# ErlerPhilipp/points2surf

Hardware: NVIDIA B200
Metric: SDF queries/sec at grid_res=256 (higher is better)
Workload: dtype f16 operands / f32 accumulate (tcgen05); hi/lo split f16 (fp32-level) for FC tails and guard-band recompute

## Files before the change

points2surf_b200/csrc/net_tc.cu:

```cuda
#include "model.cuh"
#include "tc_ptx.cuh"

#ifndef P2S_TC_BOUNDED_WAIT
#define P2S_TC_BOUNDED_WAIT 1
#endif

namespace p2s {

using namespace ptx;

namespace {

constexpr int kTile = 128;
constexpr int kThreads = 576;
constexpr uint32_t kAct2Bytes = 32768;
constexpr uint32_t kSmallBytes = 192 * 4 + 320 * 4 + 168;
template <bool PRECISE>
struct Cfg {
    static constexpr int kChunks = PRECISE ? 1 : 4;
    static constexpr int kSplit = 8 / kChunks;
    static constexpr uint32_t kChunkBytes = PRECISE ? 65536u : 32768u;
    static constexpr uint32_t kW3Bytes = kChunks * kChunkBytes;
    static constexpr uint32_t kMidBytes = (8192u + 8192u + 16384u) * (PRECISE ? 2u : 1u);
    static constexpr uint32_t kOffMid = kW3Bytes;
    static constexpr uint32_t kOffAct2 = kOffMid + kMidBytes;
    static constexpr uint32_t kOffSmall = kOffAct2 + 2 * kAct2Bytes;
    static constexpr uint32_t kSmemBytes = kOffSmall + kSmallBytes;
    static constexpr uint32_t kACols = PRECISE ? 64u : 32u;
    static constexpr uint32_t kPerqBytes = PRECISE ? 16384u : 8192u;
    static constexpr uint32_t kMidScale = PRECISE ? 2u : 1u;
};
static_assert(Cfg<false>::kSmemBytes <= 232448 && Cfg<true>::kSmemBytes <= 232448, "shared memory budget");
constexpr uint32_t kColD3 = 0;
constexpr uint32_t kColDmid = 256;
constexpr uint32_t kColDmidB = 448;
constexpr uint32_t kColA = 384;

struct Seg {
    const float* ptr;
    int n;
    int tiles;
    int center;
};

struct PassParams {
    Seg seg[2];
    const float* query;
    const float* R;
    int tiles_per_query;
    int B;
    const float* W0;
    const float* b0;
    int num_mid;
    int mid_N[3];
    const uint8_t* mid_img[3];
    const float* mid_bias[3];
    int perq_layer;
    const uint8_t* perq_img;
    const uint8_t* w3_img;
    float* out;
    long long* wstats;
};

struct Bars {
    uint64_t w_full, wq_full, perq_done;
    uint64_t dmid_free[2];
    uint64_t a_ready[2], a_free[2], dmid_ready[2];
    uint64_t act2_full[2], act2_empty[2], d3_full[2], d3_empty[2];
    uint32_t tmem_base;
};
static_assert(sizeof(Bars) <= 168, "barrier block");

__device__ __forceinline__ void wait_bar(uint64_t* bar, uint32_t parity, long long* acc = nullptr) {
#if P2S_TC_BOUNDED_WAIT
    long long t0 = clock64();
    while (!mbar_try_wait(bar, parity)) {
        if (clock64() - t0 > 2000000000LL) {
            printf("p2s: mbarrier timeout block %d thread %d bar %p parity %u\n", blockIdx.x, threadIdx.x, (void*)bar, parity);
            __trap();
        }
    }
    if (acc) *acc += clock64() - t0;
#else
    mbar_wait(bar, parity);
#endif
}
enum { WS_ACT2_FULL = 0, WS_D3_EMPTY, WS_DMID_FREE, WS_DMID_READY, WS_ACT2_EMPTY, WS_A_FREE, WS_D3_FULL, WS_TOTAL, WS_SLOTS };
__device__ __forceinline__ void ws_flush(long long* g, int role, const long long* ws, long long t_begin) {
    if (!g || (threadIdx.x & 31) != 0) return;
    for (int i = 0; i < WS_TOTAL; ++i) if (ws[i]) atomicAdd((unsigned long long*)&g[role * WS_SLOTS + i], (unsigned long long)ws[i]);
    atomicAdd((unsigned long long*)&g[role * WS_SLOTS + WS_TOTAL], (unsigned long long)(clock64() - t_begin));
}

__device__ __forceinline__ uint32_t pack_relu(float a, float b) {
    uint32_t r;
    asm("cvt.rn.relu.satfinite.f16x2.f32 %0, %1, %2;" : "=r"(r) : "f"(b), "f"(a));
    return r;
}
__device__ __forceinline__ void pack_relu_split(float a, float b, uint32_t& hi, uint32_t& lo) {
    hi = pack_relu(a, b);
    const float2 hf = __half22float2(*reinterpret_cast<const __half2*>(&hi));
    lo = pack_half2(fmaxf(a, 0.f) - hf.x, fmaxf(b, 0.f) - hf.y);
}

template <bool PRECISE, bool STATS = false>
__global__ void __launch_bounds__(kThreads, 1) pointnet_pass_kernel(const PassParams p) {
    using C = Cfg<PRECISE>;
    constexpr uint32_t kOffMid = C::kOffMid, kOffAct2 = C::kOffAct2, kOffSmall = C::kOffSmall, kOffW3 = 0;
    extern __shared__ __align__(1024) uint8_t smem[];
    float* s_wq = reinterpret_cast<float*>(smem + kOffSmall);
    float* s_bias = s_wq + 192;
    Bars* bars = reinterpret_cast<Bars*>(s_bias + 320);
    const int tid = threadIdx.x, warp = tid >> 5, lane = tid & 31;
    const int part = blockIdx.x % C::kSplit;
    const int stream = blockIdx.x / C::kSplit, nstreams = gridDim.x / C::kSplit;
    const int nq = (p.B > stream) ? (p.B - stream + nstreams - 1) / nstreams : 0;
    const int tpq = p.tiles_per_query;
    const int ntiles = nq * tpq;

    if (tid == 0) {
        mbar_init(&bars->w_full, 1);
        mbar_init(&bars->wq_full, 1);
        mbar_init(&bars->perq_done, 1);
        mbar_init(&bars->dmid_free[0], 128);
        mbar_init(&bars->dmid_free[1], 128);
        for (int i = 0; i < 2; ++i) {
            mbar_init(&bars->a_ready[i], 128);
            mbar_init(&bars->a_free[i], 128);
            mbar_init(&bars->dmid_ready[i], 1);
            mbar_init(&bars->act2_full[i], 128);
            mbar_init(&bars->act2_empty[i], 1);
            mbar_init(&bars->d3_full[i], 1);
            mbar_init(&bars->d3_empty[i], 128);
        }
        fence_mbar_init();
    }
    if (warp == 8) { tmem_alloc(&bars->tmem_base, 512); tmem_relinquish(); }
    {
        int off = 0;
        for (int l = 0; l < p.num_mid; ++l) {
            for (int i = tid; i < p.mid_N[l]; i += kThreads) s_bias[off + i] = p.mid_bias[l][i];
            off += p.mid_N[l];
        }
        for (int i = tid; i < 64; i += kThreads) s_bias[256 + i] = p.b0[i];
    }
    tc_fence_before();
    __syncthreads();
    tc_fence_after();
    const uint32_t tmem = bars->tmem_base;
    long long ws[WS_TOTAL] = {0, 0, 0, 0, 0, 0, 0};
    long long* const wsp = STATS ? ws : nullptr;
    const long long t_begin = STATS ? clock64() : 0;

    if (warp == 8) {
        if (ntiles > 0) {
            if (lane == 0) {
                uint32_t bytes = C::kW3Bytes;
                for (int l = 0; l < p.num_mid; ++l) if (l != p.perq_layer) bytes += (uint32_t)p.mid_N[l] * 128u * C::kMidScale;
                mbar_arrive_expect_tx(&bars->w_full, bytes);
                for (uint32_t o = 0; o < C::kW3Bytes; o += 32768u)
                    bulk_g2s(smem + kOffW3 + o, p.w3_img + (size_t)part * C::kW3Bytes + o, 32768, &bars->w_full);
                uint32_t o = 0;
                for (int l = 0; l < p.num_mid; ++l) {
                    const uint32_t lb = (uint32_t)p.mid_N[l] * 128u * C::kMidScale;
                    if (l != p.perq_layer) bulk_g2s(smem + kOffMid + o, p.mid_img[l], lb, &bars->w_full);
                    else {
                        mbar_arrive_expect_tx(&bars->wq_full, C::kPerqBytes);
                        bulk_g2s(smem + kOffMid + o, p.perq_img + (size_t)stream * C::kPerqBytes, C::kPerqBytes, &bars->wq_full);
                    }
                    o += lb;
                }
            }
            __syncwarp();
            wait_bar(&bars->w_full, 0);
            const uint32_t idesc_l3 = make_idesc_f16(128, 128);
            const uint64_t dsc_w3 = make_smem_desc(smem_u32(smem + kOffW3), 128, 2048);
            const uint64_t dsc_act2 = make_smem_desc(smem_u32(smem + kOffAct2), 128, 2048);
            for (int it = 0; it < ntiles; ++it) {
                const uint32_t buf = PRECISE ? 0u : ((uint32_t)it & 1), buse = PRECISE ? (uint32_t)it : ((uint32_t)it >> 1);
                wait_bar(&bars->act2_full[buf], buse & 1, wsp ? wsp + WS_ACT2_FULL : nullptr);
                const uint64_t db = dsc_act2 + (uint64_t)(buf * (kAct2Bytes >> 4));
#pragma unroll
                for (int c = 0; c < C::kChunks; ++c) {
                    const uint32_t g = (uint32_t)(it * C::kChunks + c);
                    const uint32_t stage = g & 1, use = g >> 1;
                    wait_bar(&bars->d3_empty[stage], (use & 1) ^ 1, wsp ? wsp + WS_D3_EMPTY : nullptr);
                    tc_fence_after();
                    if (elect_one()) {
                        const uint64_t da = dsc_w3 + (uint64_t)((uint32_t)c * (C::kChunkBytes >> 4));
                        const uint32_t d = tmem + kColD3 + stage * 128u;
                        if (PRECISE) {
                            const uint64_t da_lo = da + (uint64_t)(32768u >> 4), db_lo = db + (uint64_t)(32768u >> 4);
#pragma unroll
                            for (int ks = 0; ks < 8; ++ks) {
                                mma_ss(d, da_lo + (uint64_t)(ks * 16), db + (uint64_t)(ks * 16), idesc_l3, ks > 0);
                                mma_ss(d, da + (uint64_t)(ks * 16), db_lo + (uint64_t)(ks * 16), idesc_l3, 1);
                                mma_ss(d, da + (uint64_t)(ks * 16), db + (uint64_t)(ks * 16), idesc_l3, 1);
                            }
                        } else {
#pragma unroll
                            for (int ks = 0; ks < 8; ++ks)
                                mma_ss(d, da + (uint64_t)(ks * 16), db + (uint64_t)(ks * 16), idesc_l3, ks > 0);
                        }
                        mma_commit(&bars->d3_full[stage]);
                        if (c == C::kChunks - 1) mma_commit(&bars->act2_empty[buf]);
                    }
                    __syncwarp();
                }
            }
        }
    } else if (warp == 13) {
        if (ntiles > 0) {
            uint32_t mid_off[3] = {0, 0, 0};
            {
                uint32_t o = 0;
                for (int l = 0; l < p.num_mid; ++l) { mid_off[l] = o; o += (uint32_t)p.mid_N[l] * 128u * C::kMidScale; }
            }
            const bool perq = p.perq_layer >= 0;
            wait_bar(&bars->w_full, 0);
            if (perq) wait_bar(&bars->wq_full, 0);
            const uint64_t dsc_mid0 = make_smem_desc(smem_u32(smem + kOffMid) + mid_off[0], 128, 1024);
            const uint64_t dsc_mid1 = make_smem_desc(smem_u32(smem + kOffMid) + mid_off[1], 128, 1024);
            const uint64_t dsc_mid2 = make_smem_desc(smem_u32(smem + kOffMid) + mid_off[2], 128, 1024);
            const uint32_t idesc_mid0 = make_idesc_f16(128, (uint32_t)p.mid_N[0]);
            const uint32_t idesc_mid1 = make_idesc_f16(128, (uint32_t)(p.num_mid > 1 ? p.mid_N[1] : 64));
            const uint32_t idesc_mid2 = make_idesc_f16(128, (uint32_t)(p.num_mid > 2 ? p.mid_N[2] : 64));
            int it_mid0 = 0, it_mid1 = 1, l_mid0 = 0, l_mid1 = 0;
            uint32_t rnd0 = 0, rnd1 = 0;
            uint32_t g_mid = 0;
            uint32_t g_buf0 = 0, g_buf1 = 0;
            int loaded_q = 0, perq_count = 0;
            bool pq_loading = false;
            while (it_mid0 < ntiles || it_mid1 < ntiles) {
                if (perq) {
                    if (!pq_loading && perq_count == tpq && loaded_q + 1 < nq && mbar_test_wait_warp(&bars->perq_done, (uint32_t)loaded_q & 1)) {
                        if (elect_one()) {
                            mbar_arrive_expect_tx(&bars->wq_full, C::kPerqBytes);
                            bulk_g2s(smem + kOffMid + mid_off[p.perq_layer],
                                     p.perq_img + ((size_t)stream + (size_t)(loaded_q + 1) * nstreams) * C::kPerqBytes, C::kPerqBytes, &bars->wq_full);
                        }
                        __syncwarp();
                        pq_loading = true;
                    }
                    if (pq_loading && mbar_test_wait_warp(&bars->wq_full, (uint32_t)(loaded_q + 1) & 1)) {
                        ++loaded_q; perq_count = 0; pq_loading = false;
                    }
                }
                auto try_mid = [&](const int c, int& it_m, int& l_m, uint32_t& rn) {
                    if (it_m >= ntiles) return;
                    const int l = l_m;
                    if (l == p.perq_layer && it_m / tpq != loaded_q) return;
                    if (!mbar_test_wait_warp(&bars->a_ready[c], rn & 1)) return;
                    const bool small = !PRECISE && (p.mid_N[l] == 64);
                    uint32_t& g_buf = small ? g_buf1 : g_buf0;
                    if (g_buf > 0) wait_bar(&bars->dmid_free[small ? 1 : 0], (g_buf - 1) & 1, wsp ? wsp + WS_DMID_FREE : nullptr);
                    tc_fence_after();
                    const uint32_t idesc = l == 0 ? idesc_mid0 : (l == 1 ? idesc_mid1 : idesc_mid2);
                    const uint64_t dsc = l == 0 ? dsc_mid0 : (l == 1 ? dsc_mid1 : dsc_mid2);
                    const uint32_t a_t = tmem + kColA + (uint32_t)c * C::kACols;
                    const uint32_t d_t = tmem + (small ? kColDmidB : kColDmid);
                    const bool pq_last = (l == p.perq_layer) && (perq_count + 1 == tpq);
                    if (elect_one()) {
                        if (PRECISE) {
                            const uint64_t dsc_lo = dsc + (uint64_t)(((uint32_t)p.mid_N[l] * 128u) >> 4);
#pragma unroll
                            for (int ks = 0; ks < 4; ++ks) {
                                mma_ts(d_t, a_t + 32 + ks * 8, dsc + (uint64_t)(ks * 16), idesc, ks > 0);
                                mma_ts(d_t, a_t + ks * 8, dsc_lo + (uint64_t)(ks * 16), idesc, 1);
                                mma_ts(d_t, a_t + ks * 8, dsc + (uint64_t)(ks * 16), idesc, 1);
                            }
                        } else {
#pragma unroll
                            for (int ks = 0; ks < 4; ++ks)
                                mma_ts(d_t, a_t + ks * 8, dsc + (uint64_t)(ks * 16), idesc, ks > 0);
                        }
                        mma_commit(&bars->dmid_ready[c]);
                        if (pq_last) mma_commit(&bars->perq_done);
                    }
                    __syncwarp();
                    ++g_mid; ++g_buf; ++rn;
                    if (l == p.perq_layer) ++perq_count;
                    if (++l_m == p.num_mid) { l_m = 0; it_m += 2; }
                };
                if (g_mid & 1) { try_mid(1, it_mid1, l_mid1, rnd1); try_mid(0, it_mid0, l_mid0, rnd0); }
                else { try_mid(0, it_mid0, l_mid0, rnd0); try_mid(1, it_mid1, l_mid1, rnd1); }
            }
        }
    } else if (warp < 4 || (warp >= 9 && warp < 13)) {
        const int c = (warp < 4) ? 0 : 1;
        const int grp = warp & 3;
        const int pt = grp * 32 + lane;
        const uint32_t lane_base = (uint32_t)(grp * 32) << 16;
        const uint32_t a_col = tmem + lane_base + kColA + (uint32_t)c * C::kACols;
        uint32_t round = 0;
        for (int it = c; it < ntiles; it += 2) {
            const uint32_t ab = PRECISE ? 0u : (uint32_t)c;
            const uint32_t au = PRECISE ? (uint32_t)it : ((uint32_t)it >> 1);
            int boff = 0;
            for (int l = 0; l < p.num_mid; ++l, ++round) {
                wait_bar(&bars->dmid_ready[c], round & 1, wsp ? wsp + WS_DMID_READY : nullptr);
                tc_fence_after();
                const int N = p.mid_N[l];
                const bool last = (l == p.num_mid - 1);
                if (last) {
                    tc_fence_before();
                    mbar_arrive(&bars->a_free[c]);
                }
                const bool small = !PRECISE && (N == 64);
                const uint32_t dcol = small ? kColDmidB : kColDmid;
                for (int n0 = 0; n0 < N; n0 += 32) {
                    uint32_t r[32];
                    tmem_ld_x32(tmem + lane_base + dcol + n0, r);
                    tmem_ld_wait();
                    if (n0 + 32 >= N) {
                        tc_fence_before();
                        mbar_arrive(&bars->dmid_free[small ? 1 : 0]);
                    }
                    uint32_t v[16], vl[16];
#pragma unroll
                    for (int j4 = 0; j4 < 8; ++j4) {
                        const float4 bb = *reinterpret_cast<const float4*>(s_bias + boff + n0 + 4 * j4);
                        const float2 s01 = fadd2(make_float2(__uint_as_float(r[4 * j4]), __uint_as_float(r[4 * j4 + 1])), make_float2(bb.x, bb.y));
                        const float2 s23 = fadd2(make_float2(__uint_as_float(r[4 * j4 + 2]), __uint_as_float(r[4 * j4 + 3])), make_float2(bb.z, bb.w));
                        if (PRECISE) {
                            pack_relu_split(s01.x, s01.y, v[2 * j4], vl[2 * j4]);
                            pack_relu_split(s23.x, s23.y, v[2 * j4 + 1], vl[2 * j4 + 1]);
                        } else {
                            v[2 * j4] = pack_relu(s01.x, s01.y);
                            v[2 * j4 + 1] = pack_relu(s23.x, s23.y);
                        }
                    }
                    if (!last) {
                        uint32_t w[8];
#pragma unroll
                        for (int h = 0; h < 2; ++h) {
#pragma unroll
                            for (int j = 0; j < 8; ++j) w[j] = v[h * 8 + j];
                            tmem_st_x8(a_col + (uint32_t)(n0 / 2 + h * 8), w);
                            if (PRECISE) {
#pragma unroll
                                for (int j = 0; j < 8; ++j) w[j] = vl[h * 8 + j];
                                tmem_st_x8(a_col + 32u + (uint32_t)(n0 / 2 + h * 8), w);
                            }
                        }
                    } else {
                        uint8_t* dst = smem + kOffAct2 + ab * kAct2Bytes + (uint32_t)(pt >> 3) * 2048u + (uint32_t)(pt & 7) * 16u;
#pragma unroll
                        for (int j = 0; j < 4; ++j) {
                            *reinterpret_cast<uint4*>(dst + (uint32_t)(n0 / 8 + j) * 128u) = make_uint4(v[4 * j], v[4 * j + 1], v[4 * j + 2], v[4 * j + 3]);
                            if (PRECISE)
                                *reinterpret_cast<uint4*>(dst + kAct2Bytes + (uint32_t)(n0 / 8 + j) * 128u) = make_uint4(vl[4 * j], vl[4 * j + 1], vl[4 * j + 2], vl[4 * j + 3]);
                        }
                    }
                }
                if (!last) {
                    tmem_st_wait();
                    if (l == p.num_mid - 2) wait_bar(&bars->act2_empty[ab], (au & 1) ^ 1, wsp ? wsp + WS_ACT2_EMPTY : nullptr);
                    tc_fence_before();
                    mbar_arrive(&bars->a_ready[c]);
                } else {
                    fence_proxy_async_smem();
                    tc_fence_before();
                    mbar_arrive(&bars->act2_full[ab]);
                }
                boff += N;
            }
        }
    } else if (warp >= 14) {
        const int grp = warp & 3;
        const int pt = grp * 32 + lane;
        const int ct = tid - 14 * 32;
        const uint32_t lane_base = (uint32_t)(grp * 32) << 16;
        float* wq = s_wq;
        const float* s_b0 = s_bias + 256;
        int cur_q = -1;
        auto fetch = [&](int it2, float& x, float& y, float& z, float& cx, float& cy, float& cz) {
            const int qi2 = it2 / tpq, tq2 = it2 - qi2 * tpq;
            const size_t q2 = (size_t)stream + (size_t)qi2 * nstreams;
            const int sgi = tq2 < p.seg[0].tiles ? 0 : 1;
            const Seg& sg = p.seg[sgi];
            int local = (tq2 - (sgi ? p.seg[0].tiles : 0)) * kTile + pt;
            if (local >= sg.n) local = 0;
            const float* src = sg.ptr + (q2 * sg.n + local) * 3;
            x = src[0]; y = src[1]; z = src[2];
            cx = cy = cz = 0.f;
            if (sg.center) { cx = p.query[q2 * 3 + 0]; cy = p.query[q2 * 3 + 1]; cz = p.query[q2 * 3 + 2]; }
        };
        float x = 0.f, y = 0.f, z = 0.f, pcx = 0.f, pcy = 0.f, pcz = 0.f;
        if (ntiles > 0) fetch(0, x, y, z, pcx, pcy, pcz);
        for (int it = 0; it < ntiles; ++it) {
            const int c = it & 1;
            const int qi = it / tpq;
            if (qi != cur_q) {
                const size_t q = (size_t)stream + (size_t)qi * nstreams;
                asm volatile("bar.sync 3, 128;" ::: "memory");
                if (ct < 64) {
                    float w0 = p.W0[ct * 3 + 0], w1 = p.W0[ct * 3 + 1], w2 = p.W0[ct * 3 + 2];
                    float r[9] = {1.f, 0.f, 0.f, 0.f, 1.f, 0.f, 0.f, 0.f, 1.f};
                    if (p.R) {
#pragma unroll
                        for (int i = 0; i < 9; ++i) r[i] = p.R[q * 9 + i];
                    }
                    wq[0 * 64 + ct] = w0 * r[0] + w1 * r[3] + w2 * r[6];
                    wq[1 * 64 + ct] = w0 * r[1] + w1 * r[4] + w2 * r[7];
                    wq[2 * 64 + ct] = w0 * r[2] + w1 * r[5] + w2 * r[8];
                }
                asm volatile("bar.sync 3, 128;" ::: "memory");
                cur_q = qi;
            }
            x -= pcx; y -= pcy; z -= pcz;
            uint32_t v[32], vl[PRECISE ? 32 : 1];
#pragma unroll
            for (int j4 = 0; j4 < 16; ++j4) {
                const float4 wx = *reinterpret_cast<const float4*>(wq + 0 * 64 + 4 * j4);
                const float4 wy = *reinterpret_cast<const float4*>(wq + 1 * 64 + 4 * j4);
                const float4 wz = *reinterpret_cast<const float4*>(wq + 2 * 64 + 4 * j4);
                const float4 bb = *reinterpret_cast<const float4*>(s_b0 + 4 * j4);
                const float2 xx = make_float2(x, x), yy = make_float2(y, y), zz = make_float2(z, z);
                const float2 h01 = ffma2(make_float2(wx.x, wx.y), xx, ffma2(make_float2(wy.x, wy.y), yy, ffma2(make_float2(wz.x, wz.y), zz, make_float2(bb.x, bb.y))));
                const float2 h23 = ffma2(make_float2(wx.z, wx.w), xx, ffma2(make_float2(wy.z, wy.w), yy, ffma2(make_float2(wz.z, wz.w), zz, make_float2(bb.z, bb.w))));
                if (PRECISE) {
                    pack_relu_split(h01.x, h01.y, v[2 * j4], vl[2 * j4]);
                    pack_relu_split(h23.x, h23.y, v[2 * j4 + 1], vl[2 * j4 + 1]);
                } else {
                    v[2 * j4] = pack_relu(h01.x, h01.y);
                    v[2 * j4 + 1] = pack_relu(h23.x, h23.y);
                }
            }
            if (it + 1 < ntiles) fetch(it + 1, x, y, z, pcx, pcy, pcz);
            wait_bar(&bars->a_free[c], (((uint32_t)it >> 1) & 1) ^ 1, wsp ? wsp + WS_A_FREE : nullptr);
            tc_fence_after();
            tmem_st_x32(tmem + lane_base + kColA + (uint32_t)c * C::kACols, v);
            if (PRECISE) {
                uint32_t (&vl32)[32] = reinterpret_cast<uint32_t (&)[32]>(vl);
                tmem_st_x32(tmem + lane_base + kColA + (uint32_t)c * C::kACols + 32u, vl32);
            }
            tmem_st_wait();
            if (p.num_mid == 1) wait_bar(&bars->act2_empty[PRECISE ? 0 : c], ((PRECISE ? (uint32_t)it : ((uint32_t)it >> 1)) & 1) ^ 1, wsp ? wsp + WS_ACT2_EMPTY : nullptr);
            tc_fence_before();
            mbar_arrive(&bars->a_ready[c]);
        }
    } else {
        const int ew = warp - 4;
        const uint32_t lane_base = (uint32_t)(ew * 32) << 16;
        const int ch_lane = ew * 32 + lane;
        int it = 0;
        for (int qi = 0; qi < nq; ++qi) {
            const int q = stream + qi * nstreams;
            float acc[C::kChunks];
#pragma unroll
            for (int c = 0; c < C::kChunks; ++c) acc[c] = -INFINITY;
            for (int tq = 0; tq < tpq; ++tq, ++it) {
#pragma unroll
                for (int c = 0; c < C::kChunks; ++c) {
                    const uint32_t g = (uint32_t)(it * C::kChunks + c);
                    const uint32_t stage = g & 1, use = g >> 1;
                    wait_bar(&bars->d3_full[stage], use & 1, wsp ? wsp + WS_D3_FULL : nullptr);
                    tc_fence_after();
                    const uint32_t d = tmem + lane_base + kColD3 + stage * 128u;
                    float m = acc[c];
#pragma unroll
                    for (int n0 = 0; n0 < 128; n0 += 64) {
                        uint32_t r0[32], r1[32];
                        tmem_ld_x32(d + n0, r0);
                        tmem_ld_x32(d + n0 + 32, r1);
                        tmem_ld_wait();
                        if (n0 == 64) {
                            tc_fence_before();
                            mbar_arrive(&bars->d3_empty[stage]);
                        }
#pragma unroll
                        for (int j = 0; j < 32; j += 2) m = fmax3(m, __uint_as_float(r0[j]), __uint_as_float(r0[j + 1]));
#pragma unroll
                        for (int j = 0; j < 32; j += 2) m = fmax3(m, __uint_as_float(r1[j]), __uint_as_float(r1[j + 1]));
                    }
                    acc[c] = m;
                }
            }
#pragma unroll
            for (int c = 0; c < C::kChunks; ++c) p.out[(size_t)q * 1024 + (part * C::kChunks + c) * 128 + ch_lane] = acc[c];
        }
    }
    if (STATS) ws_flush(p.wstats, warp == 8 ? 0 : (warp == 13 ? 1 : (warp < 4 ? 2 : (warp >= 14 ? 4 : (warp >= 9 ? 3 : 5)))), ws, t_begin);
    tc_fence_before();
    __syncthreads();
    if (warp == 8) tmem_dealloc(tmem, 512);
}

__global__ void pack_kmajor_kernel(const float* __restrict__ W, int rows, int K, int row0, uint32_t sbo, uint8_t* __restrict__ img, int lo) {
    int e = blockIdx.x * blockDim.x + threadIdx.x;
    if (e >= rows * K) return;
    int r = e / K, k = e % K;
    uint32_t off = (uint32_t)(r >> 3) * sbo + (uint32_t)(k >> 3) * 128u + (uint32_t)(r & 7) * 16u + (uint32_t)(k & 7) * 2u;
    const float w = W[(size_t)(row0 + r) * K + k];
    const __half h = __float2half_rn(w);
    *reinterpret_cast<__half*>(img + off) = lo ? __float2half_rn(w - __half2float(h)) : h;
}

__global__ void fold_fc3_kernel(const float* __restrict__ W1, const float* __restrict__ Wfc3, const float* __restrict__ bfc3,
                                float* __restrict__ G, float* __restrict__ g0) {
    const int oi = blockIdx.x;
    const int o = oi >> 6, i = oi & 63;
    const int k = threadIdx.x;
    float acc = 0.f;
    for (int j = 0; j < 64; ++j) acc = fmaf(W1[o * 64 + j], Wfc3[(size_t)(j * 64 + i) * 256 + k], acc);
    G[(size_t)oi * 256 + k] = acc;
    if (k == 0) {
        float b = W1[o * 64 + i];
        for (int j = 0; j < 64; ++j) b = fmaf(W1[o * 64 + j], bfc3[j * 64 + i], b);
        g0[oi] = b;
    }
}

__global__ void guard_flag_kernel(const float* __restrict__ logits, int64_t B, float band, int32_t* __restrict__ list, int* __restrict__ count, int64_t base, int64_t cap) {
    int64_t i = (int64_t)blockIdx.x * blockDim.x + threadIdx.x;
    if (i >= B) return;
    if (fabsf(logits[i * 2 + 1]) < band) {
        int slot = atomicAdd(count, 1);
        if (slot < cap) list[slot] = (int32_t)(base + i);
    }
}
__global__ void guard_gather_kernel(const float* __restrict__ src, const int32_t* __restrict__ list, int n, int row_floats, float* __restrict__ dst) {
    int64_t e = (int64_t)blockIdx.x * blockDim.x + threadIdx.x;
    if (e >= (int64_t)n * row_floats) return;
    int i = (int)(e / row_floats), j = (int)(e % row_floats);
    dst[e] = src[(int64_t)list[i] * row_floats + j];
}
__global__ void guard_scatter_kernel(const float* __restrict__ src, const int32_t* __restrict__ list, int n, float* __restrict__ logits) {
    int i = blockIdx.x * blockDim.x + threadIdx.x;
    if (i >= n) return;
    logits[(int64_t)list[i] * 2 + 0] = src[i * 2 + 0];
    logits[(int64_t)list[i] * 2 + 1] = src[i * 2 + 1];
}

}

struct TcStack {
    uint8_t* w3_img = nullptr;
    uint8_t* mid_img[3] = {nullptr, nullptr, nullptr};
    uint8_t* w3_img_p = nullptr;
    uint8_t* mid_img_p[3] = {nullptr, nullptr, nullptr};
    const float* mid_bias[3] = {nullptr, nullptr, nullptr};
    int mid_N[3] = {0, 0, 0};
    int num_mid = 0;
    const float* W0 = nullptr;
    const float* b0 = nullptr;
    const float* b3 = nullptr;
};

struct TcStnFc {
    const uint8_t* fc1 = nullptr;
    const uint8_t* fc2 = nullptr;
};

struct TcWeights {
    TcStack qstn;
    TcStack stn[2], fin[2];
    TcStnFc qstn_fc, stn_fc[2];
    const uint8_t* head_fc1[2] = {nullptr, nullptr};
    const uint8_t* head_fc2 = nullptr;
    const uint8_t* head_fc3 = nullptr;
    const uint8_t* fold_img[2] = {nullptr, nullptr};
    const float* fold_bias[2] = {nullptr, nullptr};
    std::vector<void*> allocs;
    int sm_count = 148;
    bool prof_on = false;
    std::vector<std::pair<cudaEvent_t, cudaEvent_t>> prof_events;
    double prof_flops = 0.0;
    ~TcWeights() {
        for (void* a : allocs) cudaFree(a);
        for (auto& e : prof_events) { cudaEventDestroy(e.first); cudaEventDestroy(e.second); }
    }
};

namespace {

uint8_t* tc_alloc(TcWeights& t, size_t bytes) {
    void* p = nullptr;
    P2S_CUDA(cudaMalloc(&p, bytes));
    P2S_CUDA(cudaMemset(p, 0, bytes));
    t.allocs.push_back(p);
    return (uint8_t*)p;
}

uint8_t* pack_layer(TcWeights& t, const Layer& L, uint32_t sbo, bool split = false) {
    const size_t one = (size_t)L.cout * L.cin * 2;
    uint8_t* img = tc_alloc(t, one * (split ? 2 : 1));
    P2S_LAUNCH(pack_kmajor_kernel, (unsigned)cdiv((int64_t)L.cout * L.cin, 256), 256, 0, 0, L.W, L.cout, L.cin, 0, sbo, img, 0);
    if (split) P2S_LAUNCH(pack_kmajor_kernel, (unsigned)cdiv((int64_t)L.cout * L.cin, 256), 256, 0, 0, L.W, L.cout, L.cin, 0, sbo, img + one, 1);
    return img;
}

uint8_t* pack_w3(TcWeights& t, const Layer& L, bool split = false) {
    P2S_CHECK(L.cout == 1024 && L.cin == 128, "big layer must be 128 -> 1024");
    const size_t chunk = split ? 65536 : 32768;
    uint8_t* img = tc_alloc(t, 8 * chunk);
    for (int c = 0; c < 8; ++c) {
        P2S_LAUNCH(pack_kmajor_kernel, (unsigned)cdiv(128 * 128, 256), 256, 0, 0, L.W, 128, 128, c * 128, 2048u, img + (size_t)c * chunk, 0);
        if (split) P2S_LAUNCH(pack_kmajor_kernel, (unsigned)cdiv(128 * 128, 256), 256, 0, 0, L.W, 128, 128, c * 128, 2048u, img + (size_t)c * chunk + 32768, 1);
    }
    return img;
}

void launch_pass(Model& m, const TcStack& s, const Seg& s0, const Seg& s1, const float* query, const float* R,
                 int64_t B, int perq_layer, const uint8_t* perq_img, float* out, cudaStream_t st, bool precise) {
    PassParams p{};
    p.seg[0] = s0; p.seg[1] = s1;
    p.query = query; p.R = R;
    p.tiles_per_query = s0.tiles + s1.tiles;
    p.B = (int)B;
    p.W0 = s.W0; p.b0 = s.b0;
    p.num_mid = s.num_mid;
    for (int l = 0; l < 3; ++l) { p.mid_N[l] = s.mid_N[l]; p.mid_img[l] = precise ? s.mid_img_p[l] : s.mid_img[l]; p.mid_bias[l] = s.mid_bias[l]; }
    p.perq_layer = perq_layer;
    p.perq_img = perq_img;
    p.w3_img = precise ? s.w3_img_p : s.w3_img;
    p.out = out;
    p.wstats = nullptr;
    TcWeights& t = *m.tc;
    static int wstats_on = -1;
    if (wstats_on < 0) { const char* e = getenv("P2S_TC_WAITSTATS"); wstats_on = (e && e[0] == '1') ? 1 : 0; }
    static long long* wstats_dev = nullptr;
    if (wstats_on && !precise) {
        if (!wstats_dev) P2S_CUDA(cudaMalloc(&wstats_dev, 6 * WS_SLOTS * sizeof(long long)));
        P2S_CUDA(cudaMemsetAsync(wstats_dev, 0, 6 * WS_SLOTS * sizeof(long long), st));
        p.wstats = wstats_dev;
    }
    const int split = precise ? Cfg<true>::kSplit : Cfg<false>::kSplit;
    int streams = t.sm_count / split;
    if ((int64_t)streams > B) streams = (int)B;
    const int grid = streams * split;
    cudaEvent_t e0 = nullptr, e1 = nullptr;
    const bool prof = t.prof_on && !precise;
    if (prof) {
        P2S_CUDA(cudaEventCreate(&e0)); P2S_CUDA(cudaEventCreate(&e1));
        P2S_CUDA(cudaEventRecord(e0, st));
    }
    if (precise) P2S_LAUNCH(pointnet_pass_kernel<true>, grid, kThreads, Cfg<true>::kSmemBytes, st, p);
    else if (wstats_on) {
        static bool attr = false;
        if (!attr) { P2S_CUDA(cudaFuncSetAttribute(pointnet_pass_kernel<false, true>, cudaFuncAttributeMaxDynamicSharedMemorySize, (int)Cfg<false>::kSmemBytes)); attr = true; }
        P2S_LAUNCH((pointnet_pass_kernel<false, true>), grid, kThreads, Cfg<false>::kSmemBytes, st, p);
    } else P2S_LAUNCH(pointnet_pass_kernel<false>, grid, kThreads, Cfg<false>::kSmemBytes, st, p);
    if (wstats_on && !precise) {
        long long h[6 * WS_SLOTS];
        P2S_CUDA(cudaMemcpyAsync(h, wstats_dev, sizeof(h), cudaMemcpyDeviceToHost, st));
        P2S_CUDA(cudaStreamSynchronize(st));
        static const char* roles[6] = {"big-issuer", "mid-issuer", "chain0", "chain1", "first-layer", "colmax"};
        static const char* slots[WS_TOTAL] = {"act2_full", "d3_empty", "dmid_free", "dmid_ready", "act2_empty", "a_free", "d3_full"};
        fprintf(stderr, "p2s waitstats: pass num_mid=%d perq=%d pts=%d+%d B=%lld precise=%d grid=%d\n", s.num_mid, perq_layer, s0.n, s1.n, (long long)B, (int)precise, grid);
        for (int r = 0; r < 6; ++r) {
            const double tot = (double)h[r * WS_SLOTS + WS_TOTAL];
            if (tot <= 0) continue;
            fprintf(stderr, "   %-12s", roles[r]);
            for (int i = 0; i < WS_TOTAL; ++i) if (h[r * WS_SLOTS + i]) fprintf(stderr, " %s %.1f%%", slots[i], 100.0 * (double)h[r * WS_SLOTS + i] / tot);
            fprintf(stderr, "  (role cycles per warp %.0f)\n", tot / (grid * (r == 0 || r == 1 ? 1.0 : 4.0)));
        }
    }
    if (prof) {
        P2S_CUDA(cudaEventRecord(e1, st));
        t.prof_events.emplace_back(e0, e1);
        double mac_pt = 3.0 * 64 + 128.0 * 1024;
        int prev = 64;
        for (int l = 0; l < s.num_mid; ++l) { mac_pt += (double)prev * s.mid_N[l]; prev = s.mid_N[l]; }
        t.prof_flops += 2.0 * mac_pt * (double)(s0.n + s1.n) * (double)B;
    }
}

Seg make_seg(const float* ptr, int n, int center) { return Seg{ptr, n, n > 0 ? (n + kTile - 1) / kTile : 0, center}; }

}

void tc_build(Model& m) {
    P2S_CHECK(m.cfg.net_size == 1024, "tensor-core path needs net_size 1024");
    TcWeights* t = new TcWeights();
    m.tc = t;
    cudaDeviceProp prop;
    P2S_CUDA(cudaGetDeviceProperties(&prop, m.device));
    t->sm_count = prop.multiProcessorCount;
    P2S_CUDA(cudaFuncSetAttribute(pointnet_pass_kernel<false>, cudaFuncAttributeMaxDynamicSharedMemorySize, (int)Cfg<false>::kSmemBytes));
    P2S_CUDA(cudaFuncSetAttribute(pointnet_pass_kernel<true>, cudaFuncAttributeMaxDynamicSharedMemorySize, (int)Cfg<true>::kSmemBytes));
    auto build_stn = [&](TcStack& s, const Stn& stn, const Layer* c0a, const Layer* c0b) {
        if (!c0a) {
            s.W0 = stn.c1.W; s.b0 = stn.c1.b;
            s.num_mid = 1;
            s.mid_img[0] = pack_layer(*t, stn.c2, 1024); s.mid_bias[0] = stn.c2.b; s.mid_N[0] = 128;
            s.mid_img_p[0] = pack_layer(*t, stn.c2, 1024, true);
        } else {
            s.W0 = c0a->W; s.b0 = c0a->b;
            s.num_mid = 3;
            s.mid_img[0] = pack_layer(*t, *c0b, 1024); s.mid_bias[0] = c0b->b; s.mid_N[0] = 64;
            s.mid_img[1] = pack_layer(*t, stn.c1, 1024); s.mid_bias[1] = stn.c1.b; s.mid_N[1] = 64;
            s.mid_img[2] = pack_layer(*t, stn.c2, 1024); s.mid_bias[2] = stn.c2.b; s.mid_N[2] = 128;
            s.mid_img_p[0] = pack_layer(*t, *c0b, 1024, true);
            s.mid_img_p[1] = pack_layer(*t, stn.c1, 1024, true);
            s.mid_img_p[2] = pack_layer(*t, stn.c2, 1024, true);
        }
        s.w3_img_p = pack_w3(*t, stn.c3, true);
        s.w3_img = pack_w3(*t, stn.c3);
        s.b3 = stn.c3.b;
    };
    auto build_fin = [&](TcStack& s, const Feat& f) {
        s.W0 = f.conv0a.W; s.b0 = f.conv0a.b;
        s.num_mid = 3;
        s.mid_img[0] = pack_layer(*t, f.conv0b, 1024); s.mid_bias[0] = f.conv0b.b; s.mid_N[0] = 64;
        s.mid_img[1] = nullptr; s.mid_bias[1] = f.conv1.b; s.mid_N[1] = 64;
        s.mid_img[2] = pack_layer(*t, f.conv2, 1024); s.mid_bias[2] = f.conv2.b; s.mid_N[2] = 128;
        s.mid_img_p[0] = pack_layer(*t, f.conv0b, 1024, true);
        s.mid_img_p[2] = pack_layer(*t, f.conv2, 1024, true);
        s.w3_img_p = pack_w3(*t, f.conv3, true);
        s.w3_img = pack_w3(*t, f.conv3);
        s.b3 = f.conv3.b;
    };
    fc_tc_init();
    auto mk_stn_fc = [&](const Stn& s) { TcStnFc r; r.fc1 = fc_tc_pack(s.fc1, t->allocs); r.fc2 = fc_tc_pack(s.fc2, t->allocs); return r; };
    if (m.shared_qstn) t->qstn_fc = mk_stn_fc(m.point_stn);
    else if (m.global.has_qstn) t->qstn_fc = mk_stn_fc(m.global.stn1);
    t->stn_fc[0] = mk_stn_fc(m.local.stn2);
    t->stn_fc[1] = mk_stn_fc(m.global.stn2);
    for (int br = 0; br < 2; ++br) {
        const Feat& f = br ? m.global : m.local;
        P2S_CHECK(f.stn2.fc3.cout == 4096 && f.stn2.fc3.cin == 256 && f.conv1.cout == 64 && f.conv1.cin == 64, "unexpected STN shape");
        float* G = reinterpret_cast<float*>(tc_alloc(*t, (size_t)4096 * 256 * 4));
        float* g0 = reinterpret_cast<float*>(tc_alloc(*t, 4096 * 4));
        P2S_LAUNCH(fold_fc3_kernel, 4096, 256, 0, 0, f.conv1.W, f.stn2.fc3.W, f.stn2.fc3.b, G, g0);
        t->fold_img[br] = fc_tc_pack_raw(G, 4096, 256, t->allocs);
        t->fold_bias[br] = g0;
    }
    t->head_fc1[0] = fc_tc_pack(m.fc1_local, t->allocs);
    t->head_fc1[1] = fc_tc_pack(m.fc1_global, t->allocs);
    t->head_fc2 = fc_tc_pack(m.fc2, t->allocs);
    t->head_fc3 = fc_tc_pack(m.fc3, t->allocs);
    if (m.shared_qstn) build_stn(t->qstn, m.point_stn, nullptr, nullptr);
    else if (m.global.has_qstn) build_stn(t->qstn, m.global.stn1, nullptr, nullptr);
    build_stn(t->stn[0], m.local.stn2, &m.local.conv0a, &m.local.conv0b);
    build_stn(t->stn[1], m.global.stn2, &m.global.conv0a, &m.global.conv0b);
    build_fin(t->fin[0], m.local);
    build_fin(t->fin[1], m.global);
    P2S_CUDA(cudaDeviceSynchronize());
}

void tc_destroy(Model& m) {
    delete m.tc;
    m.tc = nullptr;
}

void tc_profile_reset(Model& m, bool on) {
    TcWeights& t = *m.tc;
    for (auto& e : t.prof_events) { cudaEventDestroy(e.first); cudaEventDestroy(e.second); }
    t.prof_events.clear();
    t.prof_flops = 0.0;
    t.prof_on = on;
}

void tc_profile_get(Model& m, double* ms, int64_t* launches, double* flops) {
    TcWeights& t = *m.tc;
    double total = 0.0;
    for (auto& e : t.prof_events) {
        P2S_CUDA(cudaEventSynchronize(e.second));
        float x = 0.f;
        P2S_CUDA(cudaEventElapsedTime(&x, e.first, e.second));
        total += x;
    }
    *ms = total;
    *launches = (int64_t)t.prof_events.size();
    *flops = t.prof_flops;
}

static void forward_tc_core(Model& m, const float* patch, const float* sub, const float* query, int64_t B,
                            float* logits, cudaStream_t st, bool precise) {
    TcWeights& t = *m.tc;
    const int P = m.cfg.points_per_patch, S = m.cfg.sub_sample_size;
    const int64_t Bc_max = 8192;
    const size_t per_q = 1024 + 256 + 4 + 9 + 1024 * 3 + 128 + 4096 + 1024 + 512 + 256;
    float* base = m.ws_net.as<float>(per_q * (size_t)Bc_max + 1024);
    float* pcur = base;
    auto take = [&](size_t n) { float* r = pcur; pcur += (n * (size_t)Bc_max + 63) / 64 * 64; return r; };
    float* gmax = take(1024); float* f2 = take(256); float* q4 = take(4); float* R = take(9);
    float* fmax_l = take(1024); float* fmax_g = take(1024); float* cat = take(1024); float* h4 = take(128);
    uint8_t* perq = reinterpret_cast<uint8_t*>(take(4096));
    uint8_t* imgA = reinterpret_cast<uint8_t*>(take(1024)); uint8_t* imgB = reinterpret_cast<uint8_t*>(take(512)); uint8_t* imgC = reinterpret_cast<uint8_t*>(take(256));
    auto stn_tail_img = [&](const Stn& s, const TcStnFc& f, const float* gmax_raw, int64_t Bc, float* out_f2) {
        launch_pack_a(gmax_raw, 1024, Bc, 1024, s.c3.b, true, imgA, st);
        launch_fc_tc_img(imgA, f.fc1, s.fc1.b, imgB, 0, Bc, 512, 1024, true, st, 3, 16, 0);
        if (out_f2) launch_fc_tc_img(imgB, f.fc2, s.fc2.b, out_f2, 256, Bc, 256, 512, true, st, 0);
        else launch_fc_tc_img(imgB, f.fc2, s.fc2.b, imgC, 0, Bc, 256, 512, true, st, 3, 8, 0);
    };

    for (int64_t b0 = 0; b0 < B; b0 += Bc_max) {
        const int64_t Bc = (B - b0 < Bc_max) ? (B - b0) : Bc_max;
        const float* pa = patch + b0 * P * 3;
        const float* su = sub + b0 * S * 3;
        const float* qu = query + b0 * 3;
        const float* Rq = nullptr;
        if (m.shared_qstn || m.global.has_qstn) {
            const Stn& qs = m.shared_qstn ? m.point_stn : m.global.stn1;
            const Seg s0 = m.shared_qstn ? make_seg(pa, P, 0) : make_seg(su, S, 1);
            const Seg s1 = m.shared_qstn ? make_seg(su, S, 1) : make_seg(nullptr, 0, 0);
            { StageScope ts("net: pass kernels", st); launch_pass(m, t.qstn, s0, s1, qu, nullptr, Bc, -1, nullptr, gmax, st, precise); }
            { StageScope ts("net: fc tails", st);
              stn_tail_img(qs, t.qstn_fc, gmax, Bc, f2);
              launch_gemm_nt(f2, 0, 256, qs.fc3.W, 0, qs.fc3.b, q4, 0, 4, (int)Bc, qs.fc3.cout, qs.fc3.cin, 1, false, st); }
            launch_quat_to_rot(q4, R, Bc, st);
            Rq = R;
        }
        for (int br = 1; br >= 0; --br) {
            const Feat& f = br ? m.global : m.local;
            const Seg sg = br ? make_seg(su, S, 1) : make_seg(pa, P, 0);
            float* fmax = br ? fmax_g : fmax_l;
            { StageScope ts("net: pass kernels", st); launch_pass(m, t.stn[br], sg, make_seg(nullptr, 0, 0), qu, Rq, Bc, -1, nullptr, gmax, st, precise); }
            {
                StageScope ts("net: fc tails", st);
                stn_tail_img(f.stn2, t.stn_fc[br], gmax, Bc, nullptr);
                launch_fc_tc_img(imgC, t.fold_img[br], t.fold_bias[br], perq, 0, Bc, 4096, 256, false, st, precise ? 2 : 1);
            }
            { StageScope ts("net: pass kernels", st); launch_pass(m, t.fin[br], sg, make_seg(nullptr, 0, 0), qu, Rq, Bc, 1, perq, fmax, st, precise); }
        }
        StageScope ts_head("net: fc tails", st);
        uint8_t* imgCat = reinterpret_cast<uint8_t*>(cat);
        launch_pack_a(fmax_l, 1024, Bc, 1024, m.local.conv3.b, false, imgA, st);
        launch_fc_tc_img(imgA, t.head_fc1[0], m.fc1_local.b, imgCat, 0, Bc, 512, 1024, true, st, 3, 32, 0);
        launch_pack_a(fmax_g, 1024, Bc, 1024, m.global.conv3.b, false, imgA, st);
        launch_fc_tc_img(imgA, t.head_fc1[1], m.fc1_global.b, imgCat, 0, Bc, 512, 1024, true, st, 3, 32, 16);
        if (m.debug_aux) {
            launch_bias_act(fmax_l, m.local.conv3.b, Bc, 1024, false, st);
            launch_bias_act(fmax_g, m.global.conv3.b, Bc, 1024, false, st);
            debug_aux_copy(m, b0, Bc, Rq, fmax_l, fmax_g, st);
        }
        launch_fc_tc_img(imgCat, t.head_fc2, m.fc2.b, imgC, 0, Bc, 256, 1024, true, st, 3, 8, 0);
        launch_fc_tc_img(imgC, t.head_fc3, m.fc3.b, h4, 128, Bc, 128, 256, true, st, 0);
        launch_gemm_nt(h4, 0, 128, m.fc4.W, 0, m.fc4.b, logits + b0 * 2, 0, 2, (int)Bc, 2, 128, 1, false, st);
    }
}

void forward_guard(Model& m, const float* patch, const float* sub, const float* query, int64_t B, float* logits, cudaStream_t st) {
    forward_tc_core(m, patch, sub, query, B, logits, st, true);
}

void forward_tc(Model& m, const float* patch, const float* sub, const float* query, int64_t B,
                float* logits, cudaStream_t st) {
    const int P = m.cfg.points_per_patch, S = m.cfg.sub_sample_size;
    forward_tc_core(m, patch, sub, query, B, logits, st, false);

    if (m.guard_band > 0.f && m.guard_list) {
        P2S_LAUNCH(guard_flag_kernel, (unsigned)cdiv(B, 256), 256, 0, st, logits, B, m.guard_band, m.guard_list, m.guard_list_count, m.guard_base, m.guard_list_cap);
    } else if (m.guard_band > 0.f) {
        StageScope ts_guard("net: guard-band fp32 recompute", st);
        int32_t* list = m.ws_guard.as<int32_t>((size_t)B + 64);
        int* count = reinterpret_cast<int*>(list + B);
        P2S_CUDA(cudaMemsetAsync(count, 0, sizeof(int), st));
        P2S_LAUNCH(guard_flag_kernel, (unsigned)cdiv(B, 256), 256, 0, st, logits, B, m.guard_band, list, count, (int64_t)0, B);
        int n = 0;
        P2S_CUDA(cudaMemcpyAsync(&n, count, sizeof(int), cudaMemcpyDeviceToHost, st));
        P2S_CUDA(cudaStreamSynchronize(st));
        m.last_guard_count += n;
        if (n > 0) {
            const size_t rowp = (size_t)P * 3, rows = (size_t)S * 3;
            float* gbuf = m.ws_misc.as<float>((size_t)n * (rowp + rows + 3 + 2) + 64);
            float* gp = gbuf; float* gs = gp + (size_t)n * rowp; float* gq = gs + (size_t)n * rows; float* gl = gq + ((size_t)n * 3 + 3) / 4 * 4;
            P2S_LAUNCH(guard_gather_kernel, (unsigned)cdiv((int64_t)n * rowp, 256), 256, 0, st, patch, list, n, (int)rowp, gp);
            P2S_LAUNCH(guard_gather_kernel, (unsigned)cdiv((int64_t)n * rows, 256), 256, 0, st, sub, list, n, (int)rows, gs);
            P2S_LAUNCH(guard_gather_kernel, (unsigned)cdiv((int64_t)n * 3, 256), 256, 0, st, query, list, n, 3, gq);
            forward_guard(m, gp, gs, gq, n, gl, st);
            P2S_LAUNCH(guard_scatter_kernel, (unsigned)cdiv(n, 256), 256, 0, st, gl, list, n, logits);
        }
    }
}

}
```

points2surf_b200/csrc/tc_ptx.cuh:

```cuda
#pragma once
#include <cstdint>
#include <cuda_fp16.h>

namespace p2s {
namespace ptx {

__device__ __forceinline__ uint32_t smem_u32(const void* p) { return (uint32_t)__cvta_generic_to_shared(p); }

__device__ __forceinline__ void mbar_init(uint64_t* bar, uint32_t count) {
    asm volatile("mbarrier.init.shared::cta.b64 [%0], %1;" ::"r"(smem_u32(bar)), "r"(count) : "memory");
}
__device__ __forceinline__ void fence_mbar_init() { asm volatile("fence.mbarrier_init.release.cluster;" ::: "memory"); }
__device__ __forceinline__ void mbar_arrive(uint64_t* bar) {
    asm volatile("mbarrier.arrive.shared::cta.b64 _, [%0];" ::"r"(smem_u32(bar)) : "memory");
}
__device__ __forceinline__ void mbar_arrive_expect_tx(uint64_t* bar, uint32_t bytes) {
    asm volatile("mbarrier.arrive.expect_tx.shared::cta.b64 _, [%0], %1;" ::"r"(smem_u32(bar)), "r"(bytes) : "memory");
}
__device__ __forceinline__ bool mbar_try_wait(uint64_t* bar, uint32_t parity) {
    uint32_t ok;
    asm volatile(
        "{\n\t.reg .pred p;\n\t"
        "mbarrier.try_wait.parity.shared::cta.b64 p, [%1], %2;\n\t"
        "selp.u32 %0, 1, 0, p;\n\t}"
        : "=r"(ok) : "r"(smem_u32(bar)), "r"(parity) : "memory");
    return ok != 0;
}
__device__ __forceinline__ void mbar_wait_bounded(uint64_t* bar, uint32_t parity) {
    long long t0 = clock64();
    while (!mbar_try_wait(bar, parity)) {
        if (clock64() - t0 > 2000000000LL) __trap();
    }
}
__device__ __forceinline__ bool mbar_test_wait(uint64_t* bar, uint32_t parity) {
    uint32_t ok;
    asm volatile(
        "{\n\t.reg .pred p;\n\t"
        "mbarrier.test_wait.parity.shared::cta.b64 p, [%1], %2;\n\t"
        "selp.u32 %0, 1, 0, p;\n\t}"
        : "=r"(ok) : "r"(smem_u32(bar)), "r"(parity) : "memory");
    return ok != 0;
}
__device__ __forceinline__ void mbar_wait(uint64_t* bar, uint32_t parity) {
    while (!mbar_try_wait(bar, parity)) {}
}

__device__ __forceinline__ bool mbar_test_wait_warp(uint64_t* bar, uint32_t parity) {
    return __all_sync(0xffffffffu, mbar_test_wait(bar, parity));
}
__device__ __forceinline__ bool elect_one() {
    uint32_t pred;
    asm volatile("{\n\t.reg .pred P1;\n\telect.sync _|P1, 0xffffffff;\n\tselp.u32 %0, 1, 0, P1;\n\t}" : "=r"(pred));
    return pred != 0;
}

__device__ __forceinline__ void fence_proxy_async_smem() { asm volatile("fence.proxy.async.shared::cta;" ::: "memory"); }

__device__ __forceinline__ void bulk_g2s(void* smem_dst, const void* gmem_src, uint32_t bytes, uint64_t* bar) {
    asm volatile("cp.async.bulk.shared::cluster.global.mbarrier::complete_tx::bytes [%0], [%1], %2, [%3];"
                 ::"r"(smem_u32(smem_dst)), "l"(gmem_src), "r"(bytes), "r"(smem_u32(bar)) : "memory");
}

__device__ __forceinline__ void tmem_alloc(uint32_t* smem_result, uint32_t ncols) {
    asm volatile("tcgen05.alloc.cta_group::1.sync.aligned.shared::cta.b32 [%0], %1;" ::"r"(smem_u32(smem_result)), "r"(ncols) : "memory");
}
__device__ __forceinline__ void tmem_relinquish() {
    asm volatile("tcgen05.relinquish_alloc_permit.cta_group::1.sync.aligned;" ::: "memory");
}
__device__ __forceinline__ void tmem_dealloc(uint32_t taddr, uint32_t ncols) {
    asm volatile("tcgen05.dealloc.cta_group::1.sync.aligned.b32 %0, %1;" ::"r"(taddr), "r"(ncols) : "memory");
}
__device__ __forceinline__ void tc_fence_before() { asm volatile("tcgen05.fence::before_thread_sync;" ::: "memory"); }
__device__ __forceinline__ void tc_fence_after() { asm volatile("tcgen05.fence::after_thread_sync;" ::: "memory"); }

__device__ __forceinline__ uint64_t make_smem_desc(uint32_t smem_addr, uint32_t lbo_bytes, uint32_t sbo_bytes) {
    uint64_t d = 0;
    d |= (uint64_t)((smem_addr & 0x3FFFFu) >> 4);
    d |= (uint64_t)((lbo_bytes >> 4) & 0x3FFFu) << 16;
    d |= (uint64_t)((sbo_bytes >> 4) & 0x3FFFu) << 32;
    d |= (uint64_t)1 << 46;
    return d;
}
__device__ __forceinline__ uint64_t make_smem_desc_sw128(uint32_t smem_addr) {
    uint64_t d = 0;
    d |= (uint64_t)((smem_addr & 0x3FFFFu) >> 4);
    d |= (uint64_t)1 << 16;
    d |= (uint64_t)(1024 >> 4) << 32;
    d |= (uint64_t)1 << 46;
    d |= (uint64_t)2 << 61;
    return d;
}
__host__ __device__ constexpr uint32_t make_idesc_f16(uint32_t M, uint32_t N) {
    return (1u << 4)
         | (0u << 7)
         | (0u << 10)
         | (0u << 15) | (0u << 16)
         | ((N >> 3) << 17) | ((M >> 4) << 24);
}

__device__ __forceinline__ void mma_ss(uint32_t d_tmem, uint64_t a_desc, uint64_t b_desc, uint32_t idesc, uint32_t accumulate) {
    asm volatile(
        "{\n\t.reg .pred p;\n\tsetp.ne.b32 p, %4, 0;\n\t"
        "tcgen05.mma.cta_group::1.kind::f16 [%0], %1, %2, %3, p;\n\t}"
        ::"r"(d_tmem), "l"(a_desc), "l"(b_desc), "r"(idesc), "r"(accumulate) : "memory");
}
__device__ __forceinline__ void mma_ts(uint32_t d_tmem, uint32_t a_tmem, uint64_t b_desc, uint32_t idesc, uint32_t accumulate) {
    asm volatile(
        "{\n\t.reg .pred p;\n\tsetp.ne.b32 p, %4, 0;\n\t"
        "tcgen05.mma.cta_group::1.kind::f16 [%0], [%1], %2, %3, p;\n\t}"
        ::"r"(d_tmem), "r"(a_tmem), "l"(b_desc), "r"(idesc), "r"(accumulate) : "memory");
}
__device__ __forceinline__ void mma_commit(uint64_t* bar) {
    asm volatile("tcgen05.commit.cta_group::1.mbarrier::arrive::one.shared::cluster.b64 [%0];" ::"r"(smem_u32(bar)) : "memory");
}

__device__ __forceinline__ void tmem_ld_x32(uint32_t taddr, uint32_t (&r)[32]) {
    asm volatile(
        "tcgen05.ld.sync.aligned.32x32b.x32.b32 "
        "{%0, %1, %2, %3, %4, %5, %6, %7, %8, %9, %10, %11, %12, %13, %14, %15, "
        "%16, %17, %18, %19, %20, %21, %22, %23, %24, %25, %26, %27, %28, %29, %30, %31}, [%32];"
        : "=r"(r[0]), "=r"(r[1]), "=r"(r[2]), "=r"(r[3]), "=r"(r[4]), "=r"(r[5]), "=r"(r[6]), "=r"(r[7]),
          "=r"(r[8]), "=r"(r[9]), "=r"(r[10]), "=r"(r[11]), "=r"(r[12]), "=r"(r[13]), "=r"(r[14]), "=r"(r[15]),
          "=r"(r[16]), "=r"(r[17]), "=r"(r[18]), "=r"(r[19]), "=r"(r[20]), "=r"(r[21]), "=r"(r[22]), "=r"(r[23]),
          "=r"(r[24]), "=r"(r[25]), "=r"(r[26]), "=r"(r[27]), "=r"(r[28]), "=r"(r[29]), "=r"(r[30]), "=r"(r[31])
        : "r"(taddr) : "memory");
}
__device__ __forceinline__ void tmem_ld_wait() { asm volatile("tcgen05.wait::ld.sync.aligned;" ::: "memory"); }
__device__ __forceinline__ void tmem_st_x8(uint32_t taddr, const uint32_t (&r)[8]) {
    asm volatile("tcgen05.st.sync.aligned.32x32b.x8.b32 [%0], {%1, %2, %3, %4, %5, %6, %7, %8};"
                 ::"r"(taddr), "r"(r[0]), "r"(r[1]), "r"(r[2]), "r"(r[3]), "r"(r[4]), "r"(r[5]), "r"(r[6]), "r"(r[7]) : "memory");
}
__device__ __forceinline__ void tmem_st_x32(uint32_t taddr, const uint32_t (&r)[32]) {
    asm volatile(
        "tcgen05.st.sync.aligned.32x32b.x32.b32 [%0], "
        "{%1, %2, %3, %4, %5, %6, %7, %8, %9, %10, %11, %12, %13, %14, %15, %16, "
        "%17, %18, %19, %20, %21, %22, %23, %24, %25, %26, %27, %28, %29, %30, %31, %32};"
        ::"r"(taddr), "r"(r[0]), "r"(r[1]), "r"(r[2]), "r"(r[3]), "r"(r[4]), "r"(r[5]), "r"(r[6]), "r"(r[7]),
          "r"(r[8]), "r"(r[9]), "r"(r[10]), "r"(r[11]), "r"(r[12]), "r"(r[13]), "r"(r[14]), "r"(r[15]),
          "r"(r[16]), "r"(r[17]), "r"(r[18]), "r"(r[19]), "r"(r[20]), "r"(r[21]), "r"(r[22]), "r"(r[23]),
          "r"(r[24]), "r"(r[25]), "r"(r[26]), "r"(r[27]), "r"(r[28]), "r"(r[29]), "r"(r[30]), "r"(r[31]) : "memory");
}
__device__ __forceinline__ void tmem_ld_x4(uint32_t taddr, uint32_t (&r)[4]) {
    asm volatile("tcgen05.ld.sync.aligned.32x32b.x4.b32 {%0, %1, %2, %3}, [%4];"
                 : "=r"(r[0]), "=r"(r[1]), "=r"(r[2]), "=r"(r[3]) : "r"(taddr) : "memory");
}
__device__ __forceinline__ void tmem_st_x4(uint32_t taddr, const uint32_t (&r)[4]) {
    asm volatile("tcgen05.st.sync.aligned.32x32b.x4.b32 [%0], {%1, %2, %3, %4};"
                 ::"r"(taddr), "r"(r[0]), "r"(r[1]), "r"(r[2]), "r"(r[3]) : "memory");
}
__device__ __forceinline__ void tmem_st_wait() { asm volatile("tcgen05.wait::st.sync.aligned;" ::: "memory"); }

__device__ __forceinline__ float2 fadd2(float2 a, float2 b) {
    unsigned long long ra, rb, rc;
    asm("mov.b64 %0, {%1, %2};" : "=l"(ra) : "f"(a.x), "f"(a.y));
    asm("mov.b64 %0, {%1, %2};" : "=l"(rb) : "f"(b.x), "f"(b.y));
    asm("add.rn.f32x2 %0, %1, %2;" : "=l"(rc) : "l"(ra), "l"(rb));
    float2 c;
    asm("mov.b64 {%0, %1}, %2;" : "=f"(c.x), "=f"(c.y) : "l"(rc));
    return c;
}
__device__ __forceinline__ float2 ffma2(float2 a, float2 b, float2 c) {
    unsigned long long ra, rb, rc, rd;
    asm("mov.b64 %0, {%1, %2};" : "=l"(ra) : "f"(a.x), "f"(a.y));
    asm("mov.b64 %0, {%1, %2};" : "=l"(rb) : "f"(b.x), "f"(b.y));
    asm("mov.b64 %0, {%1, %2};" : "=l"(rc) : "f"(c.x), "f"(c.y));
    asm("fma.rn.f32x2 %0, %1, %2, %3;" : "=l"(rd) : "l"(ra), "l"(rb), "l"(rc));
    float2 d;
    asm("mov.b64 {%0, %1}, %2;" : "=f"(d.x), "=f"(d.y) : "l"(rd));
    return d;
}

__device__ __forceinline__ float fmax3(float a, float b, float c) {
    float d;
    asm("max.f32 %0, %1, %2, %3;" : "=f"(d) : "f"(a), "f"(b), "f"(c));
    return d;
}
__device__ __forceinline__ uint32_t pack_half2(float lo, float hi) {
    __half2 h = __floats2half2_rn(lo, hi);
    return *reinterpret_cast<uint32_t*>(&h);
}

}
}
```

points2surf_b200/ops.py:

```python
import ctypes as C

import numpy as np
import torch

from . import _lib
from ._lib import ModelConfig, ReconConfig, P2SError, check
from . import weights as _weights


def _stream():
    return C.c_void_p(torch.cuda.current_stream().cuda_stream)


def _dev(t, dtype, name):
    if not isinstance(t, torch.Tensor) or not t.is_cuda:
        raise P2SError('%s must be a CUDA tensor (points2surf_b200 has no CPU path)' % name)
    if t.dtype != dtype:
        raise P2SError('%s must have dtype %s, got %s' % (name, dtype, t.dtype))
    return t.contiguous()


def _ptr(t):
    return C.c_void_p(t.data_ptr())


class Engine:

    def __init__(self, state_dict, use_point_stn, shared_transformer, points_per_patch=300,
                 sub_sample_size=1000, net_size=1024, device=0, precision='fp32', guard_band=0.0):
        self.lib = _lib.load()
        if not torch.cuda.is_available():
            raise P2SError('CUDA is not available: points2surf_b200 has no CPU fallback')
        self.device = torch.device('cuda', device if isinstance(device, int) else torch.device(device).index or 0)
        self.cfg = ModelConfig(int(bool(use_point_stn)), int(bool(shared_transformer)), int(points_per_patch),
                               int(sub_sample_size), int(net_size))
        blob = _weights.pack_blob(state_dict, use_point_stn, shared_transformer)
        expect = self.lib.p2s_model_blob_floats(C.byref(self.cfg))
        if blob.size != expect:
            raise P2SError('state_dict does not match the model config (%d floats, expected %d)' % (blob.size, expect))
        h = C.c_void_p()
        check(self.lib.p2s_model_create(C.byref(self.cfg), blob.ctypes.data_as(C.c_void_p), blob.size,
                                        self.device.index, C.byref(h)))
        self.handle = h
        self.P, self.S = int(points_per_patch), int(sub_sample_size)
        self.set_precision(precision, guard_band)

    def set_precision(self, precision, guard_band=0.0):
        p = {'fp32': _lib.PRECISION_FP32, 'tc': _lib.PRECISION_TC}[precision]
        check(self.lib.p2s_model_set_precision(self.handle, p, float(guard_band)))
        self.precision = precision

    def close(self):
        if getattr(self, 'handle', None):
            self.lib.p2s_model_destroy(self.handle)
            self.handle = None

    def __del__(self):
        try:
            self.close()
        except Exception:
            pass

    def forward_with_aux(self, patch_pts_ps, pts_sub_sample_ms, imp_surf_query_point_ms):
        B = patch_pts_ps.shape[0]
        aux = torch.zeros((B, 2064), dtype=torch.float32, device=patch_pts_ps.device)
        check(self.lib.p2s_model_set_debug_aux(self.handle, _ptr(aux)))
        try:
            out = self.forward(patch_pts_ps, pts_sub_sample_ms, imp_surf_query_point_ms)
            torch.cuda.synchronize()
        finally:
            check(self.lib.p2s_model_set_debug_aux(self.handle, None))
        return out, {'trans': aux[:, :9].reshape(B, 3, 3), 'feat_local_max': aux[:, 9:1033], 'feat_global_max': aux[:, 1033:2057]}

    def profile_enable(self, on=True):
        check(self.lib.p2s_profile_enable(self.handle, int(bool(on))))

    def profile_get(self):
        ms, n, fl = C.c_double(), C.c_int64(), C.c_double()
        check(self.lib.p2s_profile_get(self.handle, C.byref(ms), C.byref(n), C.byref(fl)))
        return {'ms': ms.value, 'launches': n.value, 'flops': fl.value, 'kernel': 'pointnet_pass_kernel'}

    def last_guard_count(self):
        n = C.c_int64()
        check(self.lib.p2s_model_last_guard_count(self.handle, C.byref(n)))
        return n.value

    def forward(self, patch_pts_ps, pts_sub_sample_ms, imp_surf_query_point_ms):
        pa = _dev(patch_pts_ps, torch.float32, 'patch_pts_ps')
        su = _dev(pts_sub_sample_ms, torch.float32, 'pts_sub_sample_ms')
        qu = _dev(imp_surf_query_point_ms, torch.float32, 'imp_surf_query_point_ms')
        B = pa.shape[0]
        if pa.shape != (B, self.P, 3) or su.shape != (B, self.S, 3) or qu.shape != (B, 3):
            raise P2SError('bad input shapes %s %s %s' % (tuple(pa.shape), tuple(su.shape), tuple(qu.shape)))
        out = torch.empty((B, 2), dtype=torch.float32, device=pa.device)
        if B == 0:
            return out
        with torch.cuda.device(pa.device):
            check(self.lib.p2s_forward_dev(self.handle, _ptr(pa), _ptr(su), _ptr(qu), B, _ptr(out), _stream()))
        return out

    def forward_host(self, patch_pts_ps, pts_sub_sample_ms, imp_surf_query_point_ms):
        pa = np.ascontiguousarray(patch_pts_ps, dtype=np.float32)
        su = np.ascontiguousarray(pts_sub_sample_ms, dtype=np.float32)
        qu = np.ascontiguousarray(imp_surf_query_point_ms, dtype=np.float32)
        B = pa.shape[0]
        out = np.empty((B, 2), dtype=np.float32)
        vp = lambda a: a.ctypes.data_as(C.c_void_p)
        check(self.lib.p2s_forward_host(self.handle, vp(pa), vp(su), vp(qu), B, vp(out)))
        return out

    def reconstruct(self, pts, res, eps, uniform_subsample, seed, first_query=0, num_queries=-1, batch=0, cap=None,
                    patch_radius=0.0):
        pts = _dev(pts, torch.float32, 'pts')
        N = pts.shape[0]
        if cap is None:
            cap = query_grid(pts, res, eps).numel() if num_queries < 0 else num_queries
        rc = ReconConfig(int(res), int(eps), _lib.SUBSAMPLE_UNIFORM if uniform_subsample else _lib.SUBSAMPLE_WEIGHTED,
                         int(batch), int(seed) & (2**64 - 1), float(patch_radius), 0)
        lin = torch.empty((max(cap, 1),), dtype=torch.int32, device=pts.device)
        sdf = torch.empty((max(cap, 1),), dtype=torch.float32, device=pts.device)
        Q = C.c_int64()
        with torch.cuda.device(pts.device):
            check(self.lib.p2s_reconstruct_dev(self.handle, C.byref(rc), _ptr(pts), N, int(first_query), int(num_queries),
                                               _ptr(lin), _ptr(sdf), int(cap), C.byref(Q), _stream()))
        return lin[:Q.value], sdf[:Q.value]

    def reconstruct_host(self, pts_np, res, eps, uniform_subsample, seed, cap, batch=0, out_lin=None, out_sdf=None,
                         patch_radius=0.0):
        pts_np = np.ascontiguousarray(pts_np, dtype=np.float32)
        rc = ReconConfig(int(res), int(eps), _lib.SUBSAMPLE_UNIFORM if uniform_subsample else _lib.SUBSAMPLE_WEIGHTED,
                         int(batch), int(seed) & (2**64 - 1), float(patch_radius), 0)
        lin = out_lin if out_lin is not None else np.empty((cap,), dtype=np.int32)
        sdf = out_sdf if out_sdf is not None else np.empty((cap,), dtype=np.float32)
        Q = C.c_int64()
        vp = lambda a: a.ctypes.data_as(C.c_void_p)
        check(self.lib.p2s_reconstruct_host(self.handle, C.byref(rc), vp(pts_np), pts_np.shape[0], vp(lin), vp(sdf),
                                            int(cap), C.byref(Q)))
        return lin[:Q.value], sdf[:Q.value]


def launch_count(reset=False):
    lib = _lib.load()
    n = lib.p2s_launch_count()
    if reset:
        lib.p2s_launch_count_reset()
    return int(n)


def sdf_from_logits(logits, patch_radius):
    lg = _dev(logits, torch.float32, 'logits')
    r = _dev(patch_radius, torch.float32, 'patch_radius') if patch_radius is not None else None
    out = torch.empty((lg.shape[0],), dtype=torch.float32, device=lg.device)
    with torch.cuda.device(lg.device):
        check(_lib.load().p2s_sdf_from_logits_dev(_ptr(lg), _ptr(r) if r is not None else None, lg.shape[0], _ptr(out), _stream()))
    return out


def query_grid(pts, res, eps):
    pts = _dev(pts, torch.float32, 'pts')
    lib = _lib.load()
    n = C.c_int64()
    with torch.cuda.device(pts.device):
        check(lib.p2s_query_grid_dev(_ptr(pts), pts.shape[0], int(res), int(eps), None, 0, C.byref(n), _stream()))
        out = torch.empty((max(n.value, 1),), dtype=torch.int32, device=pts.device)
        check(lib.p2s_query_grid_dev(_ptr(pts), pts.shape[0], int(res), int(eps), _ptr(out), n.value, C.byref(n), _stream()))
    return out[:n.value]


def query_points(lin_idx, res):
    lin = _dev(lin_idx, torch.int32, 'lin_idx')
    out = torch.empty((lin.shape[0], 3), dtype=torch.float32, device=lin.device)
    with torch.cuda.device(lin.device):
        check(_lib.load().p2s_query_points_dev(_ptr(lin), lin.shape[0], int(res), _ptr(out), _stream()))
    return out


def knn_patch(pts, query_pts, k):
    pts = _dev(pts, torch.float32, 'pts')
    q = _dev(query_pts, torch.float32, 'query_pts')
    Q = q.shape[0]
    ids = torch.empty((Q, k), dtype=torch.int32, device=pts.device)
    patch = torch.empty((Q, k, 3), dtype=torch.float32, device=pts.device)
    radius = torch.empty((Q,), dtype=torch.float32, device=pts.device)
    with torch.cuda.device(pts.device):
        check(_lib.load().p2s_knn_patch_dev(_ptr(pts), pts.shape[0], _ptr(q), Q, int(k), _ptr(ids), _ptr(patch),
                                            _ptr(radius), _stream()))
    return ids, patch, radius


def ball_patch(pts, query_pts, k, patch_radius, seed, query_index_base=0):
    pts = _dev(pts, torch.float32, 'pts')
    q = _dev(query_pts, torch.float32, 'query_pts')
    Q = q.shape[0]
    ids = torch.empty((Q, k), dtype=torch.int32, device=pts.device)
    patch = torch.empty((Q, k, 3), dtype=torch.float32, device=pts.device)
    radius = torch.empty((Q,), dtype=torch.float32, device=pts.device)
    counts = torch.empty((Q,), dtype=torch.int32, device=pts.device)
    with torch.cuda.device(pts.device):
        check(_lib.load().p2s_ball_patch_dev(_ptr(pts), pts.shape[0], _ptr(q), Q, int(query_index_base), int(k), float(patch_radius),
                                             int(seed) & (2**64 - 1), _ptr(ids), _ptr(patch), _ptr(radius), _ptr(counts), _stream()))
    return ids, patch, radius, counts


def subsample(pts, query_pts, S, uniform, seed, query_index_base=0):
    pts = _dev(pts, torch.float32, 'pts')
    q = _dev(query_pts, torch.float32, 'query_pts')
    Q = q.shape[0]
    ids = torch.empty((Q, S), dtype=torch.int32, device=pts.device)
    mode = _lib.SUBSAMPLE_UNIFORM if uniform else _lib.SUBSAMPLE_WEIGHTED
    with torch.cuda.device(pts.device):
        check(_lib.load().p2s_subsample_dev(_ptr(pts), pts.shape[0], _ptr(q), Q, int(query_index_base), int(S), mode,
                                            int(seed) & (2**64 - 1), _ptr(ids), _stream()))
    return ids


def gather_points(pts, ids):
    pts = _dev(pts, torch.float32, 'pts')
    ids = _dev(ids, torch.int32, 'ids')
    out = torch.empty(tuple(ids.shape) + (3,), dtype=torch.float32, device=pts.device)
    with torch.cuda.device(pts.device):
        check(_lib.load().p2s_gather_points_dev(_ptr(pts), _ptr(ids), ids.numel(), _ptr(out), _stream()))
    return out


def sdf_to_volume(lin_idx, sdf, res, sigma, certainty_threshold):
    lin = _dev(lin_idx, torch.int32, 'lin_idx')
    sd = _dev(sdf, torch.float32, 'sdf')
    vol = torch.empty((res, res, res), dtype=torch.float32, device=lin.device)
    it = C.c_int()
    with torch.cuda.device(lin.device):
        check(_lib.load().p2s_sdf_to_volume_dev(_ptr(lin), _ptr(sd), lin.shape[0], int(res), int(sigma),
                                                float(certainty_threshold), _ptr(vol), C.byref(it), _stream()))
    return vol, it.value


def marching_cubes(vol, level=0.0):
    vol = _dev(vol, torch.float32, 'vol')
    res = vol.shape[0]
    lib = _lib.load()
    nv, nf = C.c_int64(), C.c_int64()
    with torch.cuda.device(vol.device):
        check(lib.p2s_marching_cubes_dev(_ptr(vol), res, float(level), None, 0, None, 0, C.byref(nv), C.byref(nf), _stream()))
        verts = torch.empty((max(nv.value, 1), 3), dtype=torch.float32, device=vol.device)
        faces = torch.empty((max(nf.value, 1), 3), dtype=torch.int32, device=vol.device)
        check(lib.p2s_marching_cubes_dev(_ptr(vol), res, float(level), _ptr(verts), nv.value, _ptr(faces), nf.value,
                                         C.byref(nv), C.byref(nf), _stream()))
    return verts[:nv.value], faces[:nf.value]


def mesh_sample(verts, faces, num_samples, seed=0, return_face_ids=False):
    verts = _dev(verts, torch.float32, 'verts')
    faces = _dev(faces, torch.int32, 'faces')
    n = int(num_samples)
    out = torch.empty((n, 3), dtype=torch.float32, device=verts.device)
    fid = torch.empty((n,), dtype=torch.int32, device=verts.device) if return_face_ids else None
    with torch.cuda.device(verts.device):
        check(_lib.load().p2s_mesh_sample_dev(_ptr(verts), verts.shape[0], _ptr(faces), faces.shape[0], n,
                                              int(seed) & (2**64 - 1), _ptr(out), _ptr(fid) if fid is not None else None,
                                              _stream()))
    return (out, fid) if return_face_ids else out


def nn_distance(a, b):
    a = _dev(a, torch.float32, 'a')
    b = _dev(b, torch.float32, 'b')
    dist = torch.empty((a.shape[0],), dtype=torch.float32, device=a.device)
    idx = torch.empty((a.shape[0],), dtype=torch.int32, device=a.device)
    with torch.cuda.device(a.device):
        check(_lib.load().p2s_nn_distance_dev(_ptr(a), a.shape[0], _ptr(b), b.shape[0], _ptr(dist), _ptr(idx), _stream()))
    return dist, idx


def chamfer_hausdorff(a, b):
    a = _dev(a, torch.float32, 'a')
    b = _dev(b, torch.float32, 'b')
    out = (C.c_double * 4)()
    with torch.cuda.device(a.device):
        check(_lib.load().p2s_chamfer_hausdorff_dev(_ptr(a), a.shape[0], _ptr(b), b.shape[0], out, _stream()))
    return {'chamfer': out[0] + out[1], 'hausdorff_ab': out[2], 'hausdorff_ba': out[3], 'hausdorff': max(out[2], out[3])}
```

Before: 763,600.

## Move fast PointNet pass to 2-CTA cluster with cta_group::2 tcgen05 MMAs

Replaces the templated single-CTA pass kernel on the fast path with a CTA-pair cluster kernel that issues cta_group::2 tcgen05 MMAs (M=256). Each CTA now holds only half of the W3 and mid-layer weight images, and the leader CTA issues the MMAs for both. Barriers become cluster-scoped with remote arrivals. The precise path moves to a separate kernel. The aim is to halve per-CTA weight smem traffic and make better use of the tensor cores, at the cost of cross-CTA synchronization latency and possibly idle SMs if pairs do not co-schedule.

```diff
diff --git a/points2surf_b200/csrc/net_tc.cu b/points2surf_b200/csrc/net_tc.cu
--- a/points2surf_b200/csrc/net_tc.cu
+++ b/points2surf_b200/csrc/net_tc.cu
@@ -14,23 +14,16 @@
 constexpr int kTile = 128;
 constexpr int kThreads = 576;
 constexpr uint32_t kAct2Bytes = 32768;
+constexpr int kPreciseSplit = 8;
+constexpr uint32_t kPreciseChunkBytes = 65536;
+constexpr uint32_t kPreciseOffMid = kPreciseChunkBytes;
+constexpr uint32_t kPreciseOffAct2 = kPreciseOffMid + (8192u + 8192u + 16384u) * 2u;
+constexpr uint32_t kPreciseOffSmall = kPreciseOffAct2 + 2 * kAct2Bytes;
 constexpr uint32_t kSmallBytes = 192 * 4 + 320 * 4 + 168;
-template <bool PRECISE>
-struct Cfg {
-    static constexpr int kChunks = PRECISE ? 1 : 4;
-    static constexpr int kSplit = 8 / kChunks;
-    static constexpr uint32_t kChunkBytes = PRECISE ? 65536u : 32768u;
-    static constexpr uint32_t kW3Bytes = kChunks * kChunkBytes;
-    static constexpr uint32_t kMidBytes = (8192u + 8192u + 16384u) * (PRECISE ? 2u : 1u);
-    static constexpr uint32_t kOffMid = kW3Bytes;
-    static constexpr uint32_t kOffAct2 = kOffMid + kMidBytes;
-    static constexpr uint32_t kOffSmall = kOffAct2 + 2 * kAct2Bytes;
-    static constexpr uint32_t kSmemBytes = kOffSmall + kSmallBytes;
-    static constexpr uint32_t kACols = PRECISE ? 64u : 32u;
-    static constexpr uint32_t kPerqBytes = PRECISE ? 16384u : 8192u;
-    static constexpr uint32_t kMidScale = PRECISE ? 2u : 1u;
-};
-static_assert(Cfg<false>::kSmemBytes <= 232448 && Cfg<true>::kSmemBytes <= 232448, "shared memory budget");
+constexpr uint32_t kPreciseSmemBytes = kPreciseOffSmall + kSmallBytes;
+constexpr uint32_t kPreciseACols = 64;
+constexpr uint32_t kPrecisePerqBytes = 16384;
+static_assert(kPreciseSmemBytes <= 232448, "shared memory budget");
 constexpr uint32_t kColD3 = 0;
 constexpr uint32_t kColDmid = 256;
 constexpr uint32_t kColDmidB = 448;
@@ -71,18 +64,32 @@
 };
 static_assert(sizeof(Bars) <= 168, "barrier block");
 
+__device__ __noinline__ __attribute__((noreturn)) void wait_timeout(const uint64_t* bar, uint32_t parity) {
+    printf("p2s: mbarrier timeout block %d thread %d bar %p parity %u\n", blockIdx.x, threadIdx.x, (const void*)bar, parity);
+    __trap();
+}
+struct PollBound {
+    uint32_t mark = 0xffffffffu;
+    long long t0 = 0;
+    __device__ __forceinline__ void check(uint32_t m, const uint64_t* bar) {
+#if P2S_TC_BOUNDED_WAIT
+        const long long t = clock64();
+        if (m != mark) { mark = m; t0 = t; }
+        else if (t - t0 > 2000000000LL) wait_timeout(bar, m);
+#endif
+    }
+};
+template <bool CL = false>
 __device__ __forceinline__ void wait_bar(uint64_t* bar, uint32_t parity, long long* acc = nullptr) {
 #if P2S_TC_BOUNDED_WAIT
     long long t0 = clock64();
-    while (!mbar_try_wait(bar, parity)) {
-        if (clock64() - t0 > 2000000000LL) {
-            printf("p2s: mbarrier timeout block %d thread %d bar %p parity %u\n", blockIdx.x, threadIdx.x, (void*)bar, parity);
-            __trap();
-        }
+    while (!(CL ? mbar_try_wait_cluster(bar, parity) : mbar_try_wait(bar, parity))) {
+        if (clock64() - t0 > 2000000000LL) wait_timeout(bar, parity);
     }
     if (acc) *acc += clock64() - t0;
 #else
-    mbar_wait(bar, parity);
+    if (CL) { while (!mbar_try_wait_cluster(bar, parity)) {} }
+    else mbar_wait(bar, parity);
 #endif
 }
 enum { WS_ACT2_FULL = 0, WS_D3_EMPTY, WS_DMID_FREE, WS_DMID_READY, WS_ACT2_EMPTY, WS_A_FREE, WS_D3_FULL, WS_TOTAL, WS_SLOTS };
@@ -103,17 +110,404 @@
     lo = pack_half2(fmaxf(a, 0.f) - hf.x, fmaxf(b, 0.f) - hf.y);
 }
 
-template <bool PRECISE, bool STATS = false>
-__global__ void __launch_bounds__(kThreads, 1) pointnet_pass_kernel(const PassParams p) {
-    using C = Cfg<PRECISE>;
-    constexpr uint32_t kOffMid = C::kOffMid, kOffAct2 = C::kOffAct2, kOffSmall = C::kOffSmall, kOffW3 = 0;
+constexpr uint32_t kPairW3Bytes = 4 * 32768;
+constexpr uint32_t kPairMidBytes = 4096 + 8192 + 8192;
+constexpr uint32_t kPairOffMid = kPairW3Bytes;
+constexpr uint32_t kPairOffAct2 = kPairOffMid + kPairMidBytes;
+constexpr uint32_t kPairOffSmall = kPairOffAct2 + 2 * kAct2Bytes;
+constexpr uint32_t kPairSmallBytes = 192 * 4 + 320 * 4 + 176;
+constexpr uint32_t kPairSmemBytes = kPairOffSmall + kPairSmallBytes;
+static_assert(kPairSmemBytes <= 232448, "shared memory budget");
+
+struct PairBars {
+    uint64_t w_full, wq_full, perq_done;
+    uint64_t w_pair, wq_pair;
+    uint64_t dmid_free[2];
+    uint64_t a_ready[2], a_free[2], dmid_ready[2];
+    uint64_t act2_full[2], act2_empty[2], d3_full[2], d3_empty[2];
+    uint32_t tmem_base;
+};
+static_assert(sizeof(PairBars) <= 176, "barrier block");
+
+__device__ __forceinline__ uint32_t pair_mid_bytes(const PassParams& p, int l) { return l == p.perq_layer ? 8192u : (uint32_t)p.mid_N[l] * 64u; }
+
+__device__ __forceinline__ void warp_arrive_leader(uint64_t* bar) {
+    __syncwarp();
+    if ((threadIdx.x & 31) == 0) mbar_arrive_remote(bar, 0);
+}
+
+template <bool STATS = false>
+__global__ void __cluster_dims__(2, 1, 1) __launch_bounds__(kThreads, 1) pointnet_pair_kernel(const PassParams p) {
     extern __shared__ __align__(1024) uint8_t smem[];
-    float* s_wq = reinterpret_cast<float*>(smem + kOffSmall);
+    float* s_wq = reinterpret_cast<float*>(smem + kPairOffSmall);
+    float* s_bias = s_wq + 192;
+    PairBars* bars = reinterpret_cast<PairBars*>(s_bias + 320);
+    const int tid = threadIdx.x, warp = tid >> 5, lane = tid & 31;
+    const uint32_t rank = cluster_ctarank();
+    const bool leader = rank == 0;
+    const int pair = (int)(blockIdx.x >> 1), nstreams = (int)gridDim.x;
+    const int nq = (p.B - 2 * pair + nstreams - 1) / nstreams;
+    const int tpq = p.tiles_per_query;
+    const int ntiles = nq * tpq;
+    auto read_q = [&](int qi) { const int q = 2 * pair + (int)rank + qi * nstreams; return q < p.B ? q : p.B - 1; };
+    constexpr uint32_t kWarpsBoth = 8;
+
+    if (tid == 0) {
+        mbar_init(&bars->w_full, 1);
+        mbar_init(&bars->wq_full, 1);
+        mbar_init(&bars->perq_done, 1);
+        mbar_init(&bars->w_pair, 2);
+        mbar_init(&bars->wq_pair, 2);
+        mbar_init(&bars->dmid_free[0], kWarpsBoth);
+        mbar_init(&bars->dmid_free[1], kWarpsBoth);
+        for (int i = 0; i < 2; ++i) {
+            mbar_init(&bars->a_ready[i], kWarpsBoth);
+            mbar_init(&bars->a_free[i], 128);
+            mbar_init(&bars->dmid_ready[i], 1);
+            mbar_init(&bars->act2_full[i], kWarpsBoth);
+            mbar_init(&bars->act2_empty[i], 1);
+            mbar_init(&bars->d3_full[i], 1);
+            mbar_init(&bars->d3_empty[i], kWarpsBoth);
+        }
+        fence_mbar_init();
+    }
+    if (warp == 8) { tmem_alloc_pair(&bars->tmem_base, 512); tmem_relinquish_pair(); }
+    {
+        int off = 0;
+        for (int l = 0; l < p.num_mid; ++l) {
+            for (int i = tid; i < p.mid_N[l]; i += kThreads) s_bias[off + i] = p.mid_bias[l][i];
+            off += p.mid_N[l];
+        }
+        for (int i = tid; i < 64; i += kThreads) s_bias[256 + i] = p.b0[i];
+    }
+    tc_fence_before();
+    cluster_sync();
+    tc_fence_after();
+    const uint32_t tmem = bars->tmem_base;
+    long long ws[WS_TOTAL] = {0, 0, 0, 0, 0, 0, 0};
+    long long* const wsp = STATS ? ws : nullptr;
+    const long long t_begin = STATS ? clock64() : 0;
+
+    if (warp == 8) {
+        if (lane == 0) {
+            uint32_t bytes = kPairW3Bytes;
+            for (int l = 0; l < p.num_mid; ++l) if (l != p.perq_layer) bytes += pair_mid_bytes(p, l);
+            mbar_arrive_expect_tx(&bars->w_full, bytes);
+            for (int g = 0; g < 4; ++g)
+                bulk_g2s(smem + (uint32_t)g * 32768u, p.w3_img + (size_t)(2 * g + (int)rank) * 32768, 32768, &bars->w_full);
+            uint32_t o = 0;
+            for (int l = 0; l < p.num_mid; ++l) {
+                const uint32_t lb = pair_mid_bytes(p, l);
+                if (l != p.perq_layer) bulk_g2s(smem + kPairOffMid + o, p.mid_img[l] + (size_t)rank * lb, lb, &bars->w_full);
+                o += lb;
+            }
+        }
+        __syncwarp();
+        wait_bar(&bars->w_full, 0);
+        if (lane == 0) mbar_arrive_remote(&bars->w_pair, 0);
+        __syncwarp();
+        if (leader) {
+            wait_bar<true>(&bars->w_pair, 0);
+            const uint32_t idesc_l3 = make_idesc_f16(256, 128);
+            const uint64_t dsc_w3 = make_smem_desc(smem_u32(smem), 128, 2048);
+            const uint64_t dsc_act2 = make_smem_desc(smem_u32(smem + kPairOffAct2), 128, 2048);
+            for (int it = 0; it < ntiles; ++it) {
+                const uint32_t buf = (uint32_t)it & 1, buse = (uint32_t)it >> 1;
+                wait_bar<true>(&bars->act2_full[buf], buse & 1, wsp ? wsp + WS_ACT2_FULL : nullptr);
+                const uint64_t db = dsc_act2 + (uint64_t)(buf * (kAct2Bytes >> 4));
+#pragma unroll
+                for (int gh = 0; gh < 8; ++gh) {
+                    const uint32_t gc = (uint32_t)it * 8u + (uint32_t)gh;
+                    const uint32_t stage = gc & 1, use = gc >> 1;
+                    wait_bar<true>(&bars->d3_empty[stage], (use & 1) ^ 1, wsp ? wsp + WS_D3_EMPTY : nullptr);
+                    tc_fence_after();
+                    if (elect_one()) {
+                        const uint64_t da = dsc_w3 + (uint64_t)((uint32_t)(gh >> 1) * (32768u >> 4));
+                        const uint64_t dbh = db + (uint64_t)((uint32_t)(gh & 1) * (16384u >> 4));
+                        const uint32_t d = tmem + kColD3 + stage * 128u;
+#pragma unroll
+                        for (int ks = 0; ks < 8; ++ks)
+                            mma_ss_pair(d, da + (uint64_t)(ks * 16), dbh + (uint64_t)(ks * 16), idesc_l3, ks > 0);
+                        mma_commit_pair(&bars->d3_full[stage], 3);
+                        if (gh == 7) mma_commit_pair(&bars->act2_empty[buf], 3);
+                    }
+                    __syncwarp();
+                }
+            }
+        }
+    } else if (warp == 13) {
+        const uint32_t mid_off1 = pair_mid_bytes(p, 0), mid_off2 = mid_off1 + (p.num_mid > 1 ? pair_mid_bytes(p, 1) : 0u);
+        const bool perq = p.perq_layer >= 0;
+        const uint32_t perq_off = p.perq_layer == 1 ? mid_off1 : (p.perq_layer == 2 ? mid_off2 : 0u);
+        int next_q = 0;
+        bool pq_loading = false;
+        auto load_step = [&]() {
+            if (!perq || next_q >= nq) return;
+            if (!pq_loading && (next_q == 0 || mbar_test_wait_warp(&bars->perq_done, (uint32_t)(next_q - 1) & 1))) {
+                if (elect_one()) {
+                    mbar_arrive_expect_tx(&bars->wq_full, 8192);
+                    bulk_g2s(smem + kPairOffMid + perq_off, p.perq_img + (size_t)read_q(next_q) * 8192, 8192, &bars->wq_full);
+                }
+                __syncwarp();
+                pq_loading = true;
+            }
+            if (pq_loading && mbar_test_wait_warp(&bars->wq_full, (uint32_t)next_q & 1)) {
+                if (elect_one()) mbar_arrive_remote(&bars->wq_pair, 0);
+                __syncwarp();
+                pq_loading = false;
+                ++next_q;
+            }
+        };
+        if (leader) {
+            wait_bar<true>(&bars->w_pair, 0);
+            auto mid_n = [&](int l) { return l >= p.num_mid ? 64u : (l == p.perq_layer ? 128u : (uint32_t)p.mid_N[l]); };
+            const uint64_t dsc_mid0 = make_smem_desc(smem_u32(smem + kPairOffMid) + 0u, 128, 1024);
+            const uint64_t dsc_mid1 = make_smem_desc(smem_u32(smem + kPairOffMid) + mid_off1, 128, 1024);
+            const uint64_t dsc_mid2 = make_smem_desc(smem_u32(smem + kPairOffMid) + mid_off2, 128, 1024);
+            const uint32_t idesc_mid0 = make_idesc_f16(256, mid_n(0));
+            const uint32_t idesc_mid1 = make_idesc_f16(256, mid_n(1));
+            const uint32_t idesc_mid2 = make_idesc_f16(256, mid_n(2));
+            int it_mid0 = 0, it_mid1 = 1, l_mid0 = 0, l_mid1 = 0;
+            uint32_t rnd0 = 0, rnd1 = 0;
+            uint32_t g_mid = 0;
+            uint32_t g_buf0 = 0, g_buf1 = 0;
+            int perq_count = 0;
+            PollBound bound;
+            while (it_mid0 < ntiles || it_mid1 < ntiles) {
+                bound.check(g_mid + ((uint32_t)next_q << 20) + (pq_loading ? 1u << 31 : 0u), &bars->a_ready[0]);
+                load_step();
+                auto try_mid = [&](const int c, int& it_m, int& l_m, uint32_t& rn) {
+                    if (it_m >= ntiles) return;
+                    const int l = l_m;
+                    const bool pq = l == p.perq_layer;
+                    if (pq && !mbar_test_wait_warp_cluster(&bars->wq_pair, (uint32_t)(it_m / tpq) & 1)) return;
+                    if (!mbar_test_wait_warp_cluster(&bars->a_ready[c], rn & 1)) return;
+                    const bool small = !pq && p.mid_N[l] == 64;
+                    uint32_t& g_buf = small ? g_buf1 : g_buf0;
+                    if (g_buf > 0) wait_bar<true>(&bars->dmid_free[small ? 1 : 0], (g_buf - 1) & 1, wsp ? wsp + WS_DMID_FREE : nullptr);
+                    tc_fence_after();
+                    const uint32_t a_t = tmem + kColA + (uint32_t)c * 32u;
+                    const uint32_t d_t = tmem + (small ? kColDmidB : kColDmid);
+                    const bool pq_last = pq && (perq_count + 1 == tpq);
+                    const uint32_t idesc = l == 0 ? idesc_mid0 : (l == 1 ? idesc_mid1 : idesc_mid2);
+                    const uint64_t dsc = l == 0 ? dsc_mid0 : (l == 1 ? dsc_mid1 : dsc_mid2);
+                    if (elect_one()) {
+#pragma unroll
+                        for (int ks = 0; ks < 4; ++ks)
+                            mma_ts_pair(d_t, a_t + ks * 8, dsc + (uint64_t)(ks * 16), idesc, ks > 0);
+                        mma_commit_pair(&bars->dmid_ready[c], 3);
+                        if (pq_last) mma_commit_pair(&bars->perq_done, 3);
+                    }
+                    __syncwarp();
+                    ++g_mid; ++g_buf; ++rn;
+                    if (pq && ++perq_count == tpq) perq_count = 0;
+                    if (++l_m == p.num_mid) { l_m = 0; it_m += 2; }
+                };
+                if (g_mid & 1) { try_mid(1, it_mid1, l_mid1, rnd1); try_mid(0, it_mid0, l_mid0, rnd0); }
+                else { try_mid(0, it_mid0, l_mid0, rnd0); try_mid(1, it_mid1, l_mid1, rnd1); }
+            }
+        } else {
+            PollBound bound;
+            while (perq && next_q < nq) {
+                bound.check((uint32_t)next_q * 2u + (pq_loading ? 1u : 0u), &bars->wq_full);
+                load_step();
+            }
+        }
+        if (perq) wait_bar(&bars->perq_done, (uint32_t)(nq - 1) & 1);
+    } else if (warp < 4 || (warp >= 9 && warp < 13)) {
+        const int c = (warp < 4) ? 0 : 1;
+        const int grp = warp & 3;
+        const int pt = grp * 32 + lane;
+        const uint32_t lane_base = (uint32_t)(grp * 32) << 16;
+        const uint32_t a_col = tmem + lane_base + kColA + (uint32_t)c * 32u;
+        uint32_t round = 0;
+        for (int it = c; it < ntiles; it += 2) {
+            const uint32_t au = (uint32_t)it >> 1;
+            int boff = 0;
+            for (int l = 0; l < p.num_mid; ++l, ++round) {
+                wait_bar(&bars->dmid_ready[c], round & 1, wsp ? wsp + WS_DMID_READY : nullptr);
+                tc_fence_after();
+                const int N = p.mid_N[l];
+                const bool last = (l == p.num_mid - 1);
+                if (last) {
+                    tc_fence_before();
+                    mbar_arrive(&bars->a_free[c]);
+                }
+                const bool pq = l == p.perq_layer;
+                const bool small = !pq && N == 64;
+                const uint32_t dcol = (small ? kColDmidB : kColDmid) + (pq ? rank * 64u : 0u);
+                for (int n0 = 0; n0 < N; n0 += 32) {
+                    uint32_t r[32];
+                    tmem_ld_x32(tmem + lane_base + dcol + n0, r);
+                    tmem_ld_wait();
+                    if (n0 + 32 >= N) {
+                        tc_fence_before();
+                        warp_arrive_leader(&bars->dmid_free[small ? 1 : 0]);
+                    }
+                    uint32_t v[16];
+#pragma unroll
+                    for (int j4 = 0; j4 < 8; ++j4) {
+                        const float4 bb = *reinterpret_cast<const float4*>(s_bias + boff + n0 + 4 * j4);
+                        const float2 s01 = fadd2(make_float2(__uint_as_float(r[4 * j4]), __uint_as_float(r[4 * j4 + 1])), make_float2(bb.x, bb.y));
+                        const float2 s23 = fadd2(make_float2(__uint_as_float(r[4 * j4 + 2]), __uint_as_float(r[4 * j4 + 3])), make_float2(bb.z, bb.w));
+                        v[2 * j4] = pack_relu(s01.x, s01.y);
+                        v[2 * j4 + 1] = pack_relu(s23.x, s23.y);
+                    }
+                    if (!last) {
+                        uint32_t w[8];
+#pragma unroll
+                        for (int h = 0; h < 2; ++h) {
+#pragma unroll
+                            for (int j = 0; j < 8; ++j) w[j] = v[h * 8 + j];
+                            tmem_st_x8(a_col + (uint32_t)(n0 / 2 + h * 8), w);
+                        }
+                    } else {
+                        uint8_t* dst = smem + kPairOffAct2 + (uint32_t)c * kAct2Bytes + (uint32_t)(pt >> 3) * 2048u + (uint32_t)(pt & 7) * 16u;
+#pragma unroll
+                        for (int j = 0; j < 4; ++j)
+                            *reinterpret_cast<uint4*>(dst + (uint32_t)(n0 / 8 + j) * 128u) = make_uint4(v[4 * j], v[4 * j + 1], v[4 * j + 2], v[4 * j + 3]);
+                    }
+                }
+                if (!last) {
+                    tmem_st_wait();
+                    if (l == p.num_mid - 2) wait_bar(&bars->act2_empty[c], (au & 1) ^ 1, wsp ? wsp + WS_ACT2_EMPTY : nullptr);
+                    tc_fence_before();
+                    warp_arrive_leader(&bars->a_ready[c]);
+                } else {
+                    fence_proxy_async_smem();
+                    tc_fence_before();
+                    warp_arrive_leader(&bars->act2_full[c]);
+                }
+                boff += N;
+            }
+        }
+        const int n_c = (ntiles - c + 1) / 2;
+        if (n_c > 0) wait_bar(&bars->act2_empty[c], (uint32_t)(n_c - 1) & 1);
+    } else if (warp >= 14) {
+        const int grp = warp & 3;
+        const int pt = grp * 32 + lane;
+        const int ct = tid - 14 * 32;
+        const uint32_t lane_base = (uint32_t)(grp * 32) << 16;
+        float* wq = s_wq;
+        const float* s_b0 = s_bias + 256;
+        int cur_q = -1;
+        auto fetch = [&](int it2, float& x, float& y, float& z, float& cx, float& cy, float& cz) {
+            const int qi2 = it2 / tpq, tq2 = it2 - qi2 * tpq;
+            const size_t q2 = (size_t)read_q(qi2);
+            const int sgi = tq2 < p.seg[0].tiles ? 0 : 1;
+            const Seg& sg = p.seg[sgi];
+            int local = (tq2 - (sgi ? p.seg[0].tiles : 0)) * kTile + pt;
+            if (local >= sg.n) local = 0;
+            const float* src = sg.ptr + (q2 * sg.n + local) * 3;
+            x = src[0]; y = src[1]; z = src[2];
+            cx = cy = cz = 0.f;
+            if (sg.center) { cx = p.query[q2 * 3 + 0]; cy = p.query[q2 * 3 + 1]; cz = p.query[q2 * 3 + 2]; }
+        };
+        float x = 0.f, y = 0.f, z = 0.f, pcx = 0.f, pcy = 0.f, pcz = 0.f;
+        if (ntiles > 0) fetch(0, x, y, z, pcx, pcy, pcz);
+        for (int it = 0; it < ntiles; ++it) {
+            const int c = it & 1;
+            const int qi = it / tpq;
+            if (qi != cur_q) {
+                const size_t q = (size_t)read_q(qi);
+                asm volatile("bar.sync 3, 128;" ::: "memory");
+                if (ct < 64) {
+                    float w0 = p.W0[ct * 3 + 0], w1 = p.W0[ct * 3 + 1], w2 = p.W0[ct * 3 + 2];
+                    float r[9] = {1.f, 0.f, 0.f, 0.f, 1.f, 0.f, 0.f, 0.f, 1.f};
+                    if (p.R) {
+#pragma unroll
+                        for (int i = 0; i < 9; ++i) r[i] = p.R[q * 9 + i];
+                    }
+                    wq[0 * 64 + ct] = w0 * r[0] + w1 * r[3] + w2 * r[6];
+                    wq[1 * 64 + ct] = w0 * r[1] + w1 * r[4] + w2 * r[7];
+                    wq[2 * 64 + ct] = w0 * r[2] + w1 * r[5] + w2 * r[8];
+                }
+                asm volatile("bar.sync 3, 128;" ::: "memory");
+                cur_q = qi;
+            }
+            x -= pcx; y -= pcy; z -= pcz;
+            uint32_t v[32];
+#pragma unroll
+            for (int j4 = 0; j4 < 16; ++j4) {
+                const float4 wx = *reinterpret_cast<const float4*>(wq + 0 * 64 + 4 * j4);
+                const float4 wy = *reinterpret_cast<const float4*>(wq + 1 * 64 + 4 * j4);
+                const float4 wz = *reinterpret_cast<const float4*>(wq + 2 * 64 + 4 * j4);
+                const float4 bb = *reinterpret_cast<const float4*>(s_b0 + 4 * j4);
+                const float2 xx = make_float2(x, x), yy = make_float2(y, y), zz = make_float2(z, z);
+                const float2 h01 = ffma2(make_float2(wx.x, wx.y), xx, ffma2(make_float2(wy.x, wy.y), yy, ffma2(make_float2(wz.x, wz.y), zz, make_float2(bb.x, bb.y))));
+                const float2 h23 = ffma2(make_float2(wx.z, wx.w), xx, ffma2(make_float2(wy.z, wy.w), yy, ffma2(make_float2(wz.z, wz.w), zz, make_float2(bb.z, bb.w))));
+                v[2 * j4] = pack_relu(h01.x, h01.y);
+                v[2 * j4 + 1] = pack_relu(h23.x, h23.y);
+            }
+            if (it + 1 < ntiles) fetch(it + 1, x, y, z, pcx, pcy, pcz);
+            wait_bar(&bars->a_free[c], (((uint32_t)it >> 1) & 1) ^ 1, wsp ? wsp + WS_A_FREE : nullptr);
+            tc_fence_after();
+            tmem_st_x32(tmem + lane_base + kColA + (uint32_t)c * 32u, v);
+            tmem_st_wait();
+            if (p.num_mid == 1) wait_bar(&bars->act2_empty[c], (((uint32_t)it >> 1) & 1) ^ 1, wsp ? wsp + WS_ACT2_EMPTY : nullptr);
+            tc_fence_before();
+            warp_arrive_leader(&bars->a_ready[c]);
+        }
+    } else {
+        const int ew = warp - 4;
+        const uint32_t lane_base = (uint32_t)(ew * 32) << 16;
+        int it = 0;
+        for (int qi = 0; qi < nq; ++qi) {
+            float acc[2][4];
+#pragma unroll
+            for (int g = 0; g < 4; ++g) acc[0][g] = acc[1][g] = -INFINITY;
+            for (int tq = 0; tq < tpq; ++tq, ++it) {
+#pragma unroll
+                for (int gh = 0; gh < 8; ++gh) {
+                    const uint32_t gc = (uint32_t)it * 8u + (uint32_t)gh;
+                    const uint32_t stage = gc & 1, use = gc >> 1;
+                    wait_bar(&bars->d3_full[stage], use & 1, wsp ? wsp + WS_D3_FULL : nullptr);
+                    tc_fence_after();
+                    const uint32_t d = tmem + lane_base + kColD3 + stage * 128u;
+#pragma unroll
+                    for (int side = 0; side < 2; ++side) {
+                        uint32_t r0[32], r1[32];
+                        tmem_ld_x32(d + side * 64, r0);
+                        tmem_ld_x32(d + side * 64 + 32, r1);
+                        tmem_ld_wait();
+                        if (side == 1) {
+                            tc_fence_before();
+                            warp_arrive_leader(&bars->d3_empty[stage]);
+                        }
+                        float m = acc[side][gh >> 1];
+#pragma unroll
+                        for (int j = 0; j < 32; j += 2) m = fmax3(m, __uint_as_float(r0[j]), __uint_as_float(r0[j + 1]));
+#pragma unroll
+                        for (int j = 0; j < 32; j += 2) m = fmax3(m, __uint_as_float(r1[j]), __uint_as_float(r1[j + 1]));
+                        acc[side][gh >> 1] = m;
+                    }
+                }
+            }
+            const int q0 = 2 * pair + qi * nstreams;
+#pragma unroll
+            for (int side = 0; side < 2; ++side) {
+                if (q0 + side >= p.B) continue;
+#pragma unroll
+                for (int g = 0; g < 4; ++g) p.out[(size_t)(q0 + side) * 1024 + g * 256 + (int)rank * 128 + ew * 32 + lane] = acc[side][g];
+            }
+        }
+    }
+    if (STATS && (leader || (warp != 8 && warp != 13)))
+        ws_flush(p.wstats, warp == 8 ? 0 : (warp == 13 ? 1 : (warp < 4 ? 2 : (warp >= 14 ? 4 : (warp >= 9 ? 3 : 5)))), ws, t_begin);
+    tc_fence_before();
+    cluster_sync();
+    tc_fence_after();
+    if (warp == 8) tmem_dealloc_pair(tmem, 512);
+}
+
+__global__ void __launch_bounds__(kThreads, 1) pointnet_pass_precise_kernel(const PassParams p) {
+    extern __shared__ __align__(1024) uint8_t smem[];
+    float* s_wq = reinterpret_cast<float*>(smem + kPreciseOffSmall);
     float* s_bias = s_wq + 192;
     Bars* bars = reinterpret_cast<Bars*>(s_bias + 320);
     const int tid = threadIdx.x, warp = tid >> 5, lane = tid & 31;
-    const int part = blockIdx.x % C::kSplit;
-    const int stream = blockIdx.x / C::kSplit, nstreams = gridDim.x / C::kSplit;
+    const int part = blockIdx.x % kPreciseSplit;
+    const int stream = blockIdx.x / kPreciseSplit, nstreams = gridDim.x / kPreciseSplit;
     const int nq = (p.B > stream) ? (p.B - stream + nstreams - 1) / nstreams : 0;
     const int tpq = p.tiles_per_query;
     const int ntiles = nq * tpq;
@@ -148,25 +542,22 @@
     __syncthreads();
     tc_fence_after();
     const uint32_t tmem = bars->tmem_base;
-    long long ws[WS_TOTAL] = {0, 0, 0, 0, 0, 0, 0};
-    long long* const wsp = STATS ? ws : nullptr;
-    const long long t_begin = STATS ? clock64() : 0;
 
     if (warp == 8) {
         if (ntiles > 0) {
             if (lane == 0) {
-                uint32_t bytes = C::kW3Bytes;
-                for (int l = 0; l < p.num_mid; ++l) if (l != p.perq_layer) bytes += (uint32_t)p.mid_N[l] * 128u * C::kMidScale;
+                uint32_t bytes = kPreciseChunkBytes;
+                for (int l = 0; l < p.num_mid; ++l) if (l != p.perq_layer) bytes += (uint32_t)p.mid_N[l] * 256u;
                 mbar_arrive_expect_tx(&bars->w_full, bytes);
-                for (uint32_t o = 0; o < C::kW3Bytes; o += 32768u)
-                    bulk_g2s(smem + kOffW3 + o, p.w3_img + (size_t)part * C::kW3Bytes + o, 32768, &bars->w_full);
+                for (uint32_t o = 0; o < kPreciseChunkBytes; o += 32768u)
+                    bulk_g2s(smem + o, p.w3_img + (size_t)part * kPreciseChunkBytes + o, 32768, &bars->w_full);
                 uint32_t o = 0;
                 for (int l = 0; l < p.num_mid; ++l) {
-                    const uint32_t lb = (uint32_t)p.mid_N[l] * 128u * C::kMidScale;
-                    if (l != p.perq_layer) bulk_g2s(smem + kOffMid + o, p.mid_img[l], lb, &bars->w_full);
+                    const uint32_t lb = (uint32_t)p.mid_N[l] * 256u;
+                    if (l != p.perq_layer) bulk_g2s(smem + kPreciseOffMid + o, p.mid_img[l], lb, &bars->w_full);
                     else {
-                        mbar_arrive_expect_tx(&bars->wq_full, C::kPerqBytes);
-                        bulk_g2s(smem + kOffMid + o, p.perq_img + (size_t)stream * C::kPerqBytes, C::kPerqBytes, &bars->wq_full);
+                        mbar_arrive_expect_tx(&bars->wq_full, kPrecisePerqBytes);
+                        bulk_g2s(smem + kPreciseOffMid + o, p.perq_img + (size_t)stream * kPrecisePerqBytes, kPrecisePerqBytes, &bars->wq_full);
                     }
                     o += lb;
                 }
@@ -174,39 +565,26 @@
             __syncwarp();
             wait_bar(&bars->w_full, 0);
             const uint32_t idesc_l3 = make_idesc_f16(128, 128);
-            const uint64_t dsc_w3 = make_smem_desc(smem_u32(smem + kOffW3), 128, 2048);
-            const uint64_t dsc_act2 = make_smem_desc(smem_u32(smem + kOffAct2), 128, 2048);
+            const uint64_t dsc_w3 = make_smem_desc(smem_u32(smem), 128, 2048);
+            const uint64_t db = make_smem_desc(smem_u32(smem + kPreciseOffAct2), 128, 2048);
             for (int it = 0; it < ntiles; ++it) {
-                const uint32_t buf = PRECISE ? 0u : ((uint32_t)it & 1), buse = PRECISE ? (uint32_t)it : ((uint32_t)it >> 1);
-                wait_bar(&bars->act2_full[buf], buse & 1, wsp ? wsp + WS_ACT2_FULL : nullptr);
-                const uint64_t db = dsc_act2 + (uint64_t)(buf * (kAct2Bytes >> 4));
-#pragma unroll
-                for (int c = 0; c < C::kChunks; ++c) {
-                    const uint32_t g = (uint32_t)(it * C::kChunks + c);
-                    const uint32_t stage = g & 1, use = g >> 1;
-                    wait_bar(&bars->d3_empty[stage], (use & 1) ^ 1, wsp ? wsp + WS_D3_EMPTY : nullptr);
-                    tc_fence_after();
-                    if (elect_one()) {
-                        const uint64_t da = dsc_w3 + (uint64_t)((uint32_t)c * (C::kChunkBytes >> 4));
-                        const uint32_t d = tmem + kColD3 + stage * 128u;
-                        if (PRECISE) {
-                            const uint64_t da_lo = da + (uint64_t)(32768u >> 4), db_lo = db + (uint64_t)(32768u >> 4);
-#pragma unroll
-                            for (int ks = 0; ks < 8; ++ks) {
-                                mma_ss(d, da_lo + (uint64_t)(ks * 16), db + (uint64_t)(ks * 16), idesc_l3, ks > 0);
-                                mma_ss(d, da + (uint64_t)(ks * 16), db_lo + (uint64_t)(ks * 16), idesc_l3, 1);
-                                mma_ss(d, da + (uint64_t)(ks * 16), db + (uint64_t)(ks * 16), idesc_l3, 1);
-                            }
-                        } else {
-#pragma unroll
-                            for (int ks = 0; ks < 8; ++ks)
-                                mma_ss(d, da + (uint64_t)(ks * 16), db + (uint64_t)(ks * 16), idesc_l3, ks > 0);
-                        }
-                        mma_commit(&bars->d3_full[stage]);
-                        if (c == C::kChunks - 1) mma_commit(&bars->act2_empty[buf]);
-                    }
-                    __syncwarp();
-                }
+                const uint32_t stage = (uint32_t)it & 1, use = (uint32_t)it >> 1;
+                wait_bar(&bars->act2_full[0], (uint32_t)it & 1);
+                wait_bar(&bars->d3_empty[stage], (use & 1) ^ 1);
+                tc_fence_after();
+                if (elect_one()) {
+                    const uint32_t d = tmem + kColD3 + stage * 128u;
+                    const uint64_t da_lo = dsc_w3 + (uint64_t)(32768u >> 4), db_lo = db + (uint64_t)(32768u >> 4);
+#pragma unroll
+                    for (int ks = 0; ks < 8; ++ks) {
+                        mma_ss(d, da_lo + (uint64_t)(ks * 16), db + (uint64_t)(ks * 16), idesc_l3, ks > 0);
+                        mma_ss(d, dsc_w3 + (uint64_t)(ks * 16), db_lo + (uint64_t)(ks * 16), idesc_l3, 1);
+                        mma_ss(d, dsc_w3 + (uint64_t)(ks * 16), db + (uint64_t)(ks * 16), idesc_l3, 1);
+                    }
+                    mma_commit(&bars->d3_full[stage]);
+                    mma_commit(&bars->act2_empty[0]);
+                }
+                __syncwarp();
             }
         }
     } else if (warp == 13) {
@@ -214,30 +592,32 @@
             uint32_t mid_off[3] = {0, 0, 0};
             {
                 uint32_t o = 0;
-                for (int l = 0; l < p.num_mid; ++l) { mid_off[l] = o; o += (uint32_t)p.mid_N[l] * 128u * C::kMidScale; }
+                for (int l = 0; l < p.num_mid; ++l) { mid_off[l] = o; o += (uint32_t)p.mid_N[l] * 256u; }
             }
             const bool perq = p.perq_layer >= 0;
             wait_bar(&bars->w_full, 0);
             if (perq) wait_bar(&bars->wq_full, 0);
-            const uint64_t dsc_mid0 = make_smem_desc(smem_u32(smem + kOffMid) + mid_off[0], 128, 1024);
-            const uint64_t dsc_mid1 = make_smem_desc(smem_u32(smem + kOffMid) + mid_off[1], 128, 1024);
-            const uint64_t dsc_mid2 = make_smem_desc(smem_u32(smem + kOffMid) + mid_off[2], 128, 1024);
+            const uint64_t dsc_mid0 = make_smem_desc(smem_u32(smem + kPreciseOffMid) + mid_off[0], 128, 1024);
+            const uint64_t dsc_mid1 = make_smem_desc(smem_u32(smem + kPreciseOffMid) + mid_off[1], 128, 1024);
+            const uint64_t dsc_mid2 = make_smem_desc(smem_u32(smem + kPreciseOffMid) + mid_off[2], 128, 1024);
             const uint32_t idesc_mid0 = make_idesc_f16(128, (uint32_t)p.mid_N[0]);
             const uint32_t idesc_mid1 = make_idesc_f16(128, (uint32_t)(p.num_mid > 1 ? p.mid_N[1] : 64));
             const uint32_t idesc_mid2 = make_idesc_f16(128, (uint32_t)(p.num_mid > 2 ? p.mid_N[2] : 64));
             int it_mid0 = 0, it_mid1 = 1, l_mid0 = 0, l_mid1 = 0;
             uint32_t rnd0 = 0, rnd1 = 0;
             uint32_t g_mid = 0;
-            uint32_t g_buf0 = 0, g_buf1 = 0;
+            uint32_t g_buf = 0;
             int loaded_q = 0, perq_count = 0;
             bool pq_loading = false;
+            PollBound bound;
             while (it_mid0 < ntiles || it_mid1 < ntiles) {
+                bound.check(g_mid + ((uint32_t)loaded_q << 20) + (pq_loading ? 1u << 31 : 0u), &bars->a_ready[0]);
                 if (perq) {
                     if (!pq_loading && perq_count == tpq && loaded_q + 1 < nq && mbar_test_wait_warp(&bars->perq_done, (uint32_t)loaded_q & 1)) {
                         if (elect_one()) {
-                            mbar_arrive_expect_tx(&bars->wq_full, C::kPerqBytes);
-                            bulk_g2s(smem + kOffMid + mid_off[p.perq_layer],
-                                     p.perq_img + ((size_t)stream + (size_t)(loaded_q + 1) * nstreams) * C::kPerqBytes, C::kPerqBytes, &bars->wq_full);
+                            mbar_arrive_expect_tx(&bars->wq_full, kPrecisePerqBytes);
+                            bulk_g2s(smem + kPreciseOffMid + mid_off[p.perq_layer],
+                                     p.perq_img + ((size_t)stream + (size_t)(loaded_q + 1) * nstreams) * kPrecisePerqBytes, kPrecisePerqBytes, &bars->wq_full);
                         }
                         __syncwarp();
                         pq_loading = true;
@@ -251,28 +631,20 @@
                     const int l = l_m;
                     if (l == p.perq_layer && it_m / tpq != loaded_q) return;
                     if (!mbar_test_wait_warp(&bars->a_ready[c], rn & 1)) return;
-                    const bool small = !PRECISE && (p.mid_N[l] == 64);
-                    uint32_t& g_buf = small ? g_buf1 : g_buf0;
-                    if (g_buf > 0) wait_bar(&bars->dmid_free[small ? 1 : 0], (g_buf - 1) & 1, wsp ? wsp + WS_DMID_FREE : nullptr);
+                    if (g_buf > 0) wait_bar(&bars->dmid_free[0], (g_buf - 1) & 1);
                     tc_fence_after();
                     const uint32_t idesc = l == 0 ? idesc_mid0 : (l == 1 ? idesc_mid1 : idesc_mid2);
                     const uint64_t dsc = l == 0 ? dsc_mid0 : (l == 1 ? dsc_mid1 : dsc_mid2);
-                    const uint32_t a_t = tmem + kColA + (uint32_t)c * C::kACols;
-                    const uint32_t d_t = tmem + (small ? kColDmidB : kColDmid);
+                    const uint32_t a_t = tmem + kColA + (uint32_t)c * kPreciseACols;
+                    const uint32_t d_t = tmem + kColDmid;
                     const bool pq_last = (l == p.perq_layer) && (perq_count + 1 == tpq);
                     if (elect_one()) {
-                        if (PRECISE) {
-                            const uint64_t dsc_lo = dsc + (uint64_t)(((uint32_t)p.mid_N[l] * 128u) >> 4);
-#pragma unroll
-                            for (int ks = 0; ks < 4; ++ks) {
-                                mma_ts(d_t, a_t + 32 + ks * 8, dsc + (uint64_t)(ks * 16), idesc, ks > 0);
-                                mma_ts(d_t, a_t + ks * 8, dsc_lo + (uint64_t)(ks * 16), idesc, 1);
-                                mma_ts(d_t, a_t + ks * 8, dsc + (uint64_t)(ks * 16), idesc, 1);
-                            }
-                        } else {
-#pragma unroll
-                            for (int ks = 0; ks < 4; ++ks)
-                                mma_ts(d_t, a_t + ks * 8, dsc + (uint64_t)(ks * 16), idesc, ks > 0);
+                        const uint64_t dsc_lo = dsc + (uint64_t)(((uint32_t)p.mid_N[l] * 128u) >> 4);
+#pragma unroll
+                        for (int ks = 0; ks < 4; ++ks) {
+                            mma_ts(d_t, a_t + 32 + ks * 8, dsc + (uint64_t)(ks * 16), idesc, ks > 0);
+                            mma_ts(d_t, a_t + ks * 8, dsc_lo + (uint64_t)(ks * 16), idesc, 1);
+                            mma_ts(d_t, a_t + ks * 8, dsc + (uint64_t)(ks * 16), idesc, 1);
                         }
                         mma_commit(&bars->dmid_ready[c]);
                         if (pq_last) mma_commit(&bars->perq_done);
@@ -291,14 +663,12 @@
         const int grp = warp & 3;
         const int pt = grp * 32 + lane;
         const uint32_t lane_base = (uint32_t)(grp * 32) << 16;
-        const uint32_t a_col = tmem + lane_base + kColA + (uint32_t)c * C::kACols;
+        const uint32_t a_col = tmem + lane_base + kColA + (uint32_t)c * kPreciseACols;
         uint32_t round = 0;
         for (int it = c; it < ntiles; it += 2) {
-            const uint32_t ab = PRECISE ? 0u : (uint32_t)c;
-            const uint32_t au = PRECISE ? (uint32_t)it : ((uint32_t)it >> 1);
             int boff = 0;
             for (int l = 0; l < p.num_mid; ++l, ++round) {
-                wait_bar(&bars->dmid_ready[c], round & 1, wsp ? wsp + WS_DMID_READY : nullptr);
+                wait_bar(&bars->dmid_ready[c], round & 1);
                 tc_fence_after();
                 const int N = p.mid_N[l];
                 const bool last = (l == p.num_mid - 1);
@@ -306,15 +676,13 @@
                     tc_fence_before();
                     mbar_arrive(&bars->a_free[c]);
                 }
-                const bool small = !PRECISE && (N == 64);
-                const uint32_t dcol = small ? kColDmidB : kColDmid;
                 for (int n0 = 0; n0 < N; n0 += 32) {
                     uint32_t r[32];
-                    tmem_ld_x32(tmem + lane_base + dcol + n0, r);
+                    tmem_ld_x32(tmem + lane_base + kColDmid + n0, r);
                     tmem_ld_wait();
                     if (n0 + 32 >= N) {
                         tc_fence_before();
-                        mbar_arrive(&bars->dmid_free[small ? 1 : 0]);
+                        mbar_arrive(&bars->dmid_free[0]);
                     }
                     uint32_t v[16], vl[16];
 #pragma unroll
@@ -322,13 +690,8 @@
                         const float4 bb = *reinterpret_cast<const float4*>(s_bias + boff + n0 + 4 * j4);
                         const float2 s01 = fadd2(make_float2(__uint_as_float(r[4 * j4]), __uint_as_float(r[4 * j4 + 1])), make_float2(bb.x, bb.y));
                         const float2 s23 = fadd2(make_float2(__uint_as_float(r[4 * j4 + 2]), __uint_as_float(r[4 * j4 + 3])), make_float2(bb.z, bb.w));
-                        if (PRECISE) {
-                            pack_relu_split(s01.x, s01.y, v[2 * j4], vl[2 * j4]);
-                            pack_relu_split(s23.x, s23.y, v[2 * j4 + 1], vl[2 * j4 + 1]);
-                        } else {
-                            v[2 * j4] = pack_relu(s01.x, s01.y);
-                            v[2 * j4 + 1] = pack_relu(s23.x, s23.y);
-                        }
+                        pack_relu_split(s01.x, s01.y, v[2 * j4], vl[2 * j4]);
+                        pack_relu_split(s23.x, s23.y, v[2 * j4 + 1], vl[2 * j4 + 1]);
                     }
                     if (!last) {
                         uint32_t w[8];
@@ -337,31 +700,28 @@
 #pragma unroll
                             for (int j = 0; j < 8; ++j) w[j] = v[h * 8 + j];
                             tmem_st_x8(a_col + (uint32_t)(n0 / 2 + h * 8), w);
-                            if (PRECISE) {
-#pragma unroll
-                                for (int j = 0; j < 8; ++j) w[j] = vl[h * 8 + j];
-                                tmem_st_x8(a_col + 32u + (uint32_t)(n0 / 2 + h * 8), w);
-                            }
+#pragma unroll
+                            for (int j = 0; j < 8; ++j) w[j] = vl[h * 8 + j];
+                            tmem_st_x8(a_col + 32u + (uint32_t)(n0 / 2 + h * 8), w);
                         }
                     } else {
-                        uint8_t* dst = smem + kOffAct2 + ab * kAct2Bytes + (uint32_t)(pt >> 3) * 2048u + (uint32_t)(pt & 7) * 16u;
+                        uint8_t* dst = smem + kPreciseOffAct2 + (uint32_t)(pt >> 3) * 2048u + (uint32_t)(pt & 7) * 16u;
 #pragma unroll
                         for (int j = 0; j < 4; ++j) {
                             *reinterpret_cast<uint4*>(dst + (uint32_t)(n0 / 8 + j) * 128u) = make_uint4(v[4 * j], v[4 * j + 1], v[4 * j + 2], v[4 * j + 3]);
-                            if (PRECISE)
-                                *reinterpret_cast<uint4*>(dst + kAct2Bytes + (uint32_t)(n0 / 8 + j) * 128u) = make_uint4(vl[4 * j], vl[4 * j + 1], vl[4 * j + 2], vl[4 * j + 3]);
+                            *reinterpret_cast<uint4*>(dst + kAct2Bytes + (uint32_t)(n0 / 8 + j) * 128u) = make_uint4(vl[4 * j], vl[4 * j + 1], vl[4 * j + 2], vl[4 * j + 3]);
                         }
                     }
                 }
                 if (!last) {
                     tmem_st_wait();
-                    if (l == p.num_mid - 2) wait_bar(&bars->act2_empty[ab], (au & 1) ^ 1, wsp ? wsp + WS_ACT2_EMPTY : nullptr);
+                    if (l == p.num_mid - 2) wait_bar(&bars->act2_empty[0], ((uint32_t)it & 1) ^ 1);
                     tc_fence_before();
                     mbar_arrive(&bars->a_ready[c]);
                 } else {
                     fence_proxy_async_smem();
                     tc_fence_before();
-                    mbar_arrive(&bars->act2_full[ab]);
+                    mbar_arrive(&bars->act2_full[0]);
                 }
                 boff += N;
             }
@@ -409,7 +769,7 @@
                 cur_q = qi;
             }
             x -= pcx; y -= pcy; z -= pcz;
-            uint32_t v[32], vl[PRECISE ? 32 : 1];
+            uint32_t v[32], vl[32];
 #pragma unroll
             for (int j4 = 0; j4 < 16; ++j4) {
                 const float4 wx = *reinterpret_cast<const float4*>(wq + 0 * 64 + 4 * j4);
@@ -419,24 +779,16 @@
                 const float2 xx = make_float2(x, x), yy = make_float2(y, y), zz = make_float2(z, z);
                 const float2 h01 = ffma2(make_float2(wx.x, wx.y), xx, ffma2(make_float2(wy.x, wy.y), yy, ffma2(make_float2(wz.x, wz.y), zz, make_float2(bb.x, bb.y))));
                 const float2 h23 = ffma2(make_float2(wx.z, wx.w), xx, ffma2(make_float2(wy.z, wy.w), yy, ffma2(make_float2(wz.z, wz.w), zz, make_float2(bb.z, bb.w))));
-                if (PRECISE) {
-                    pack_relu_split(h01.x, h01.y, v[2 * j4], vl[2 * j4]);
-                    pack_relu_split(h23.x, h23.y, v[2 * j4 + 1], vl[2 * j4 + 1]);
-                } else {
-                    v[2 * j4] = pack_relu(h01.x, h01.y);
-                    v[2 * j4 + 1] = pack_relu(h23.x, h23.y);
-                }
+                pack_relu_split(h01.x, h01.y, v[2 * j4], vl[2 * j4]);
+                pack_relu_split(h23.x, h23.y, v[2 * j4 + 1], vl[2 * j4 + 1]);
             }
             if (it + 1 < ntiles) fetch(it + 1, x, y, z, pcx, pcy, pcz);
-            wait_bar(&bars->a_free[c], (((uint32_t)it >> 1) & 1) ^ 1, wsp ? wsp + WS_A_FREE : nullptr);
+            wait_bar(&bars->a_free[c], (((uint32_t)it >> 1) & 1) ^ 1);
             tc_fence_after();
-            tmem_st_x32(tmem + lane_base + kColA + (uint32_t)c * C::kACols, v);
-            if (PRECISE) {
-                uint32_t (&vl32)[32] = reinterpret_cast<uint32_t (&)[32]>(vl);
-                tmem_st_x32(tmem + lane_base + kColA + (uint32_t)c * C::kACols + 32u, vl32);
-            }
+            tmem_st_x32(tmem + lane_base + kColA + (uint32_t)c * kPreciseACols, v);
+            tmem_st_x32(tmem + lane_base + kColA + (uint32_t)c * kPreciseACols + 32u, vl);
             tmem_st_wait();
-            if (p.num_mid == 1) wait_bar(&bars->act2_empty[PRECISE ? 0 : c], ((PRECISE ? (uint32_t)it : ((uint32_t)it >> 1)) & 1) ^ 1, wsp ? wsp + WS_ACT2_EMPTY : nullptr);
+            if (p.num_mid == 1) wait_bar(&bars->act2_empty[0], ((uint32_t)it & 1) ^ 1);
             tc_fence_before();
             mbar_arrive(&bars->a_ready[c]);
         }
@@ -447,41 +799,31 @@
         int it = 0;
         for (int qi = 0; qi < nq; ++qi) {
             const int q = stream + qi * nstreams;
-            float acc[C::kChunks];
-#pragma unroll
-            for (int c = 0; c < C::kChunks; ++c) acc[c] = -INFINITY;
+            float acc = -INFINITY;
             for (int tq = 0; tq < tpq; ++tq, ++it) {
-#pragma unroll
-                for (int c = 0; c < C::kChunks; ++c) {
-                    const uint32_t g = (uint32_t)(it * C::kChunks + c);
-                    const uint32_t stage = g & 1, use = g >> 1;
-                    wait_bar(&bars->d3_full[stage], use & 1, wsp ? wsp + WS_D3_FULL : nullptr);
-                    tc_fence_after();
-                    const uint32_t d = tmem + lane_base + kColD3 + stage * 128u;
-                    float m = acc[c];
-#pragma unroll
-                    for (int n0 = 0; n0 < 128; n0 += 64) {
-                        uint32_t r0[32], r1[32];
-                        tmem_ld_x32(d + n0, r0);
-                        tmem_ld_x32(d + n0 + 32, r1);
-                        tmem_ld_wait();
-                        if (n0 == 64) {
-                            tc_fence_before();
-                            mbar_arrive(&bars->d3_empty[stage]);
-                        }
-#pragma unroll
-                        for (int j = 0; j < 32; j += 2) m = fmax3(m, __uint_as_float(r0[j]), __uint_as_float(r0[j + 1]));
-#pragma unroll
-                        for (int j = 0; j < 32; j += 2) m = fmax3(m, __uint_as_float(r1[j]), __uint_as_float(r1[j + 1]));
-                    }
-                    acc[c] = m;
-                }
-            }
-#pragma unroll
-            for (int c = 0; c < C::kChunks; ++c) p.out[(size_t)q * 1024 + (part * C::kChunks + c) * 128 + ch_lane] = acc[c];
-        }
-    }
-    if (STATS) ws_flush(p.wstats, warp == 8 ? 0 : (warp == 13 ? 1 : (warp < 4 ? 2 : (warp >= 14 ? 4 : (warp >= 9 ? 3 : 5)))), ws, t_begin);
+                const uint32_t stage = (uint32_t)it & 1, use = (uint32_t)it >> 1;
+                wait_bar(&bars->d3_full[stage], use & 1);
+                tc_fence_after();
+                const uint32_t d = tmem + lane_base + kColD3 + stage * 128u;
+#pragma unroll
+                for (int n0 = 0; n0 < 128; n0 += 64) {
+                    uint32_t r0[32], r1[32];
+                    tmem_ld_x32(d + n0, r0);
+                    tmem_ld_x32(d + n0 + 32, r1);
+                    tmem_ld_wait();
+                    if (n0 == 64) {
+                        tc_fence_before();
+                        mbar_arrive(&bars->d3_empty[stage]);
+                    }
+#pragma unroll
+                    for (int j = 0; j < 32; j += 2) acc = fmax3(acc, __uint_as_float(r0[j]), __uint_as_float(r0[j + 1]));
+#pragma unroll
+                    for (int j = 0; j < 32; j += 2) acc = fmax3(acc, __uint_as_float(r1[j]), __uint_as_float(r1[j + 1]));
+                }
+            }
+            p.out[(size_t)q * 1024 + part * 128 + ch_lane] = acc;
+        }
+    }
     tc_fence_before();
     __syncthreads();
     if (warp == 8) tmem_dealloc(tmem, 512);
@@ -564,6 +906,7 @@
     const float* fold_bias[2] = {nullptr, nullptr};
     std::vector<void*> allocs;
     int sm_count = 148;
+    int pair_clusters = 74;
     bool prof_on = false;
     std::vector<std::pair<cudaEvent_t, cudaEvent_t>> prof_events;
     double prof_flops = 0.0;
@@ -626,35 +969,39 @@
         P2S_CUDA(cudaMemsetAsync(wstats_dev, 0, 6 * WS_SLOTS * sizeof(long long), st));
         p.wstats = wstats_dev;
     }
-    const int split = precise ? Cfg<true>::kSplit : Cfg<false>::kSplit;
-    int streams = t.sm_count / split;
-    if ((int64_t)streams > B) streams = (int)B;
-    const int grid = streams * split;
+    int grid;
+    if (precise) {
+        int streams = t.sm_count / kPreciseSplit;
+        if ((int64_t)streams > B) streams = (int)B;
+        grid = streams * kPreciseSplit;
+    } else {
+        grid = 2 * (int)std::min<int64_t>(t.pair_clusters, (B + 1) / 2);
+    }
     cudaEvent_t e0 = nullptr, e1 = nullptr;
     const bool prof = t.prof_on && !precise;
     if (prof) {
         P2S_CUDA(cudaEventCreate(&e0)); P2S_CUDA(cudaEventCreate(&e1));
         P2S_CUDA(cudaEventRecord(e0, st));
     }
-    if (precise) P2S_LAUNCH(pointnet_pass_kernel<true>, grid, kThreads, Cfg<true>::kSmemBytes, st, p);
+    if (precise) P2S_LAUNCH(pointnet_pass_precise_kernel, grid, kThreads, kPreciseSmemBytes, st, p);
     else if (wstats_on) {
         static bool attr = false;
-        if (!attr) { P2S_CUDA(cudaFuncSetAttribute(pointnet_pass_kernel<false, true>, cudaFuncAttributeMaxDynamicSharedMemorySize, (int)Cfg<false>::kSmemBytes)); attr = true; }
-        P2S_LAUNCH((pointnet_pass_kernel<false, true>), grid, kThreads, Cfg<false>::kSmemBytes, st, p);
-    } else P2S_LAUNCH(pointnet_pass_kernel<false>, grid, kThreads, Cfg<false>::kSmemBytes, st, p);
+        if (!attr) { P2S_CUDA(cudaFuncSetAttribute(pointnet_pair_kernel<true>, cudaFuncAttributeMaxDynamicSharedMemorySize, (int)kPairSmemBytes)); attr = true; }
+        P2S_LAUNCH(pointnet_pair_kernel<true>, grid, kThreads, kPairSmemBytes, st, p);
+    } else P2S_LAUNCH(pointnet_pair_kernel<false>, grid, kThreads, kPairSmemBytes, st, p);
     if (wstats_on && !precise) {
         long long h[6 * WS_SLOTS];
         P2S_CUDA(cudaMemcpyAsync(h, wstats_dev, sizeof(h), cudaMemcpyDeviceToHost, st));
         P2S_CUDA(cudaStreamSynchronize(st));
-        static const char* roles[6] = {"big-issuer", "mid-issuer", "chain0", "chain1", "first-layer", "colmax"};
+        static const char* roles[6] = {"pair-big-issuer", "pair-mid-issuer", "chain0", "chain1", "first-layer", "colmax"};
         static const char* slots[WS_TOTAL] = {"act2_full", "d3_empty", "dmid_free", "dmid_ready", "act2_empty", "a_free", "d3_full"};
-        fprintf(stderr, "p2s waitstats: pass num_mid=%d perq=%d pts=%d+%d B=%lld precise=%d grid=%d\n", s.num_mid, perq_layer, s0.n, s1.n, (long long)B, (int)precise, grid);
+        fprintf(stderr, "p2s waitstats: pass num_mid=%d perq=%d pts=%d+%d B=%lld grid=%d (CTA pairs)\n", s.num_mid, perq_layer, s0.n, s1.n, (long long)B, grid);
         for (int r = 0; r < 6; ++r) {
             const double tot = (double)h[r * WS_SLOTS + WS_TOTAL];
             if (tot <= 0) continue;
-            fprintf(stderr, "   %-12s", roles[r]);
+            fprintf(stderr, "   %-16s", roles[r]);
             for (int i = 0; i < WS_TOTAL; ++i) if (h[r * WS_SLOTS + i]) fprintf(stderr, " %s %.1f%%", slots[i], 100.0 * (double)h[r * WS_SLOTS + i] / tot);
-            fprintf(stderr, "  (role cycles per warp %.0f)\n", tot / (grid * (r == 0 || r == 1 ? 1.0 : 4.0)));
+            fprintf(stderr, "  (role cycles per warp %.0f)\n", tot / (r == 0 || r == 1 ? grid / 2.0 : grid * 4.0));
         }
     }
     if (prof) {
@@ -678,8 +1025,20 @@
     cudaDeviceProp prop;
     P2S_CUDA(cudaGetDeviceProperties(&prop, m.device));
     t->sm_count = prop.multiProcessorCount;
-    P2S_CUDA(cudaFuncSetAttribute(pointnet_pass_kernel<false>, cudaFuncAttributeMaxDynamicSharedMemorySize, (int)Cfg<false>::kSmemBytes));
-    P2S_CUDA(cudaFuncSetAttribute(pointnet_pass_kernel<true>, cudaFuncAttributeMaxDynamicSharedMemorySize, (int)Cfg<true>::kSmemBytes));
+    P2S_CUDA(cudaFuncSetAttribute(pointnet_pair_kernel<false>, cudaFuncAttributeMaxDynamicSharedMemorySize, (int)kPairSmemBytes));
+    P2S_CUDA(cudaFuncSetAttribute(pointnet_pass_precise_kernel, cudaFuncAttributeMaxDynamicSharedMemorySize, (int)kPreciseSmemBytes));
+    {
+        cudaLaunchConfig_t cfg = {};
+        cfg.gridDim = dim3((unsigned)(2 * (t->sm_count / 2)));
+        cfg.blockDim = dim3(kThreads);
+        cfg.dynamicSmemBytes = kPairSmemBytes;
+        int clusters = 0;
+        P2S_CUDA(cudaOccupancyMaxActiveClusters(&clusters, (void*)pointnet_pair_kernel<false>, &cfg));
+        P2S_CHECK(clusters > 0, "the pass kernel's CTA pair does not fit on this GPU");
+        t->pair_clusters = clusters;
+        if (2 * clusters < t->sm_count)
+            fprintf(stderr, "p2s: %d CTA pairs co-resident, %d of %d SMs idle in the pass kernel\n", clusters, t->sm_count - 2 * clusters, t->sm_count);
+    }
     auto build_stn = [&](TcStack& s, const Stn& stn, const Layer* c0a, const Layer* c0b) {
         if (!c0a) {
             s.W0 = stn.c1.W; s.b0 = stn.c1.b;
diff --git a/points2surf_b200/csrc/tc_ptx.cuh b/points2surf_b200/csrc/tc_ptx.cuh
--- a/points2surf_b200/csrc/tc_ptx.cuh
+++ b/points2surf_b200/csrc/tc_ptx.cuh
@@ -45,8 +45,46 @@
     while (!mbar_try_wait(bar, parity)) {}
 }
 
+__device__ __forceinline__ bool mbar_try_wait_cluster(uint64_t* bar, uint32_t parity) {
+    uint32_t ok;
+    asm volatile(
+        "{\n\t.reg .pred p;\n\t"
+        "mbarrier.try_wait.parity.acquire.cluster.shared::cta.b64 p, [%1], %2;\n\t"
+        "selp.u32 %0, 1, 0, p;\n\t}"
+        : "=r"(ok) : "r"(smem_u32(bar)), "r"(parity) : "memory");
+    return ok != 0;
+}
+__device__ __forceinline__ bool mbar_test_wait_cluster(uint64_t* bar, uint32_t parity) {
+    uint32_t ok;
+    asm volatile(
+        "{\n\t.reg .pred p;\n\t"
+        "mbarrier.test_wait.parity.acquire.cluster.shared::cta.b64 p, [%1], %2;\n\t"
+        "selp.u32 %0, 1, 0, p;\n\t}"
+        : "=r"(ok) : "r"(smem_u32(bar)), "r"(parity) : "memory");
+    return ok != 0;
+}
+__device__ __forceinline__ void mbar_arrive_remote(uint64_t* bar, uint32_t cta) {
+    asm volatile(
+        "{\n\t.reg .b32 ra;\n\t"
+        "mapa.shared::cluster.u32 ra, %0, %1;\n\t"
+        "mbarrier.arrive.release.cluster.shared::cluster.b64 _, [ra];\n\t}"
+        ::"r"(smem_u32(bar)), "r"(cta) : "memory");
+}
+
 __device__ __forceinline__ bool mbar_test_wait_warp(uint64_t* bar, uint32_t parity) {
     return __all_sync(0xffffffffu, mbar_test_wait(bar, parity));
+}
+__device__ __forceinline__ bool mbar_test_wait_warp_cluster(uint64_t* bar, uint32_t parity) {
+    return __all_sync(0xffffffffu, mbar_test_wait_cluster(bar, parity));
+}
+
+__device__ __forceinline__ uint32_t cluster_ctarank() {
+    uint32_t r;
+    asm volatile("mov.u32 %0, %%cluster_ctarank;" : "=r"(r));
+    return r;
+}
+__device__ __forceinline__ void cluster_sync() {
+    asm volatile("barrier.cluster.arrive.release.aligned;\n\tbarrier.cluster.wait.acquire.aligned;" ::: "memory");
 }
 __device__ __forceinline__ bool elect_one() {
     uint32_t pred;
@@ -69,6 +107,15 @@
 }
 __device__ __forceinline__ void tmem_dealloc(uint32_t taddr, uint32_t ncols) {
     asm volatile("tcgen05.dealloc.cta_group::1.sync.aligned.b32 %0, %1;" ::"r"(taddr), "r"(ncols) : "memory");
+}
+__device__ __forceinline__ void tmem_alloc_pair(uint32_t* smem_result, uint32_t ncols) {
+    asm volatile("tcgen05.alloc.cta_group::2.sync.aligned.shared::cta.b32 [%0], %1;" ::"r"(smem_u32(smem_result)), "r"(ncols) : "memory");
+}
+__device__ __forceinline__ void tmem_relinquish_pair() {
+    asm volatile("tcgen05.relinquish_alloc_permit.cta_group::2.sync.aligned;" ::: "memory");
+}
+__device__ __forceinline__ void tmem_dealloc_pair(uint32_t taddr, uint32_t ncols) {
+    asm volatile("tcgen05.dealloc.cta_group::2.sync.aligned.b32 %0, %1;" ::"r"(taddr), "r"(ncols) : "memory");
 }
 __device__ __forceinline__ void tc_fence_before() { asm volatile("tcgen05.fence::before_thread_sync;" ::: "memory"); }
 __device__ __forceinline__ void tc_fence_after() { asm volatile("tcgen05.fence::after_thread_sync;" ::: "memory"); }
@@ -112,6 +159,23 @@
 }
 __device__ __forceinline__ void mma_commit(uint64_t* bar) {
     asm volatile("tcgen05.commit.cta_group::1.mbarrier::arrive::one.shared::cluster.b64 [%0];" ::"r"(smem_u32(bar)) : "memory");
+}
+
+__device__ __forceinline__ void mma_ss_pair(uint32_t d_tmem, uint64_t a_desc, uint64_t b_desc, uint32_t idesc, uint32_t accumulate) {
+    asm volatile(
+        "{\n\t.reg .pred p;\n\tsetp.ne.b32 p, %4, 0;\n\t"
+        "tcgen05.mma.cta_group::2.kind::f16 [%0], %1, %2, %3, p;\n\t}"
+        ::"r"(d_tmem), "l"(a_desc), "l"(b_desc), "r"(idesc), "r"(accumulate) : "memory");
+}
+__device__ __forceinline__ void mma_ts_pair(uint32_t d_tmem, uint32_t a_tmem, uint64_t b_desc, uint32_t idesc, uint32_t accumulate) {
+    asm volatile(
+        "{\n\t.reg .pred p;\n\tsetp.ne.b32 p, %4, 0;\n\t"
+        "tcgen05.mma.cta_group::2.kind::f16 [%0], [%1], %2, %3, p;\n\t}"
+        ::"r"(d_tmem), "r"(a_tmem), "l"(b_desc), "r"(idesc), "r"(accumulate) : "memory");
+}
+__device__ __forceinline__ void mma_commit_pair(uint64_t* bar, uint16_t cta_mask) {
+    asm volatile("tcgen05.commit.cta_group::2.mbarrier::arrive::one.shared::cluster.multicast::cluster.b64 [%0], %1;"
+                 ::"r"(smem_u32(bar)), "h"(cta_mask) : "memory");
 }
 
 __device__ __forceinline__ void tmem_ld_x32(uint32_t taddr, uint32_t (&r)[32]) {
diff --git a/points2surf_b200/ops.py b/points2surf_b200/ops.py
--- a/points2surf_b200/ops.py
+++ b/points2surf_b200/ops.py
@@ -78,7 +78,7 @@
     def profile_get(self):
         ms, n, fl = C.c_double(), C.c_int64(), C.c_double()
         check(self.lib.p2s_profile_get(self.handle, C.byref(ms), C.byref(n), C.byref(fl)))
-        return {'ms': ms.value, 'launches': n.value, 'flops': fl.value, 'kernel': 'pointnet_pass_kernel'}
+        return {'ms': ms.value, 'launches': n.value, 'flops': fl.value, 'kernel': 'pointnet_pair_kernel'}
 
     def last_guard_count(self):
         n = C.c_int64()
```

Measured after the change: 834,300 (median of 6 runs). +9.3%, better.
